# GewelsJI/MVLT

Measured on AMD Instinct MI355X. Metric: image-text pairs/sec/node, PVT-tiny MVLT pre-train step, higher is better.
Workload: dtype bf16

## Files before the change

### include/mvlt_hip.h

```cpp
#ifndef MVLT_HIP_H
#define MVLT_HIP_H
#include <stdint.h>
#ifdef __cplusplus
extern "C" {
#endif

#define MVLT_DT_BF16 0
#define MVLT_DT_FP32 1

#define MVLT_ABI_VERSION 7
const char* mvlt_last_error(void);
int mvlt_abi_version(void);
const char* mvlt_last_kernel(void);
int mvlt_sizeof(const char* name);

typedef struct mvlt_rowmap {
  int mode, rows_per_batch, batch_stride, offset;
  int r, w_in, tokens_in, hw_out, w_out, c_seg;
  int h_in;
} mvlt_rowmap;

typedef struct mvlt_gemm_nt_args {
  const void* A; const void* B; void* C;
  int M, N, K, lda, ldb, ldc;
  int dtype;
  int out_dtype;
  mvlt_rowmap a_map, c_map;
  const float* bias;
  int act;
  void* H;
  const float* row_scale;
  int rows_per_scale;
  const void* R;
  float* col_sum;
  float* col_sumsq;
  int col_copies;
  int split_k;
  void* post_y; int post_ld;
  const float* post_gamma; const float* post_beta; float post_eps;
  float* post_mean; float* post_rstd;
  int r_fp32;
} mvlt_gemm_nt_args;
int mvlt_gemm_nt(const mvlt_gemm_nt_args* args, void* stream);

typedef struct mvlt_gemm_tn_args {
  const void* A; const void* B; float* C;
  int M, N1, N2, lda, ldb, ldc;
  int dtype;
  mvlt_rowmap a_map, b_map;
  float* colsum_a;
  int splits;
  float* colsum_b;
  int trans_c;
  int c_taps, c_seg;
  const void* dgrad_wt; void* dgrad_out; int dgrad_ld;
  void* partials; long partials_bytes;
  int defer_fold;
  int c_overwrite;
} mvlt_gemm_tn_args;
int mvlt_gemm_tn(const mvlt_gemm_tn_args* args, void* stream);
int mvlt_tn_fold_flush(const void* partials, void* stream);
int mvlt_tn_fold_discard(const void* partials);

typedef struct mvlt_layernorm_args {
  const void* x; void* y;
  const float* gamma; const float* beta;
  float* mean; float* rstd;
  const float* add;
  int add_rows;
  int rows, C, ldx, ldy;
  mvlt_rowmap x_map, y_map;
  float eps;
  int dtype;
  int y_dtype;
  void* y2; const float* gamma2; const float* beta2; float eps2; float* mean2; float* rstd2;
} mvlt_layernorm_args;
int mvlt_layernorm_fwd(const mvlt_layernorm_args* args, void* stream);

typedef struct mvlt_layernorm_bwd_args {
  const void* dy; const void* x; void* dx;
  const float* gamma; const float* mean; const float* rstd;
  float* dgamma; float* dbeta;
  int rows, C, lddy, ldx, lddx;
  mvlt_rowmap dy_map, x_map, dx_map;
  int dx_accumulate;
  int dtype;
  int x_dtype, dx_dtype;
  void* dx2; const float* dx2_scale; int dx2_rows_per_scale; int lddx2;
  int dg_copies; long dg_copy_stride;
} mvlt_layernorm_bwd_args;
int mvlt_layernorm_bwd(const mvlt_layernorm_bwd_args* args, void* stream);
int mvlt_fold_copies(float* arena, int copies, long stride, const int* dst_index, int j0, int j1, float* dst, void* stream);

int mvlt_batch_sum(const void* in, float* out, int B, int R, int C, long batch_stride_rows, int ld, int dtype,
                   float* acc2 , int split, void* stream);

typedef struct mvlt_attn_args {
  const void* Q; const void* KV; void* O; float* lse;
  int B, H, N, M;
  int ldq, ldkv, ldo;
  int k_off, v_off;
  float scale;
  int dtype;
} mvlt_attn_args;
int mvlt_sr_attention_fwd(const mvlt_attn_args* args, void* stream);

typedef struct mvlt_attn_bwd_args {
  const void* Q; const void* KV; const void* O; const void* dO; const float* lse;
  void* dQ; void* dKV;
  int B, H, N, M;
  int ldq, ldkv, ldo, lddkv;
  int k_off, v_off;
  float scale;
  int dtype;
  int dkv_dtype;
} mvlt_attn_bwd_args;
int mvlt_sr_attention_bwd(const mvlt_attn_bwd_args* args, void* stream);
int mvlt_sr_attention_bwd_chunks(int B, int H, int N, int M, int dtype);
int mvlt_sr_attention_fwd_streamed(const mvlt_attn_args* args, void* stream);
int mvlt_sr_attention_bwd_streamed(const mvlt_attn_bwd_args* args, void* stream);


int mvlt_bert_embed_fwd(const long* ids, const float* word, const float* pos, const float* type0, const float* gamma,
                        const float* beta, const uint8_t* keep, float drop_p, void* y, float* mean, float* rstd,
                        int rows, int T, int hidden, float eps, int dtype, void* stream);
int mvlt_bert_embed_bwd(const void* dy, const long* ids, const float* word, const float* pos, const float* type0,
                        const float* gamma, const uint8_t* keep, float drop_p, const float* mean, const float* rstd,
                        float* dword, float* dpos, float* dtype0, float* dgamma, float* dbeta,
                        int rows, int T, int hidden, int dtype, void* stream);

int mvlt_patchify(const float* img, void* out, int B, int Cin, int H, int W, int k, int dtype, void* stream);

int mvlt_masked_select(const long* labels, int n, long ignore_index, int* idx, int* count, void* stream);

int mvlt_resize_bilinear_tokens(const float* in, int ld_in, float* out, int ld_out, int Hin, int Win, int Hout, int Wout, int C, int adjoint,
                                void* stream);
int mvlt_resize_bilinear_tokens_multi(const float* const* in, const int* ld_in, float* const* out, const int* ld_out, const int* Hin, const int* Win,
                                      const int* Hout, const int* Wout, const int* C, int count, int adjoint, void* stream);

int mvlt_gelu_bwd(const void* dy, const void* h, void* out, long n, int dtype, void* stream);
int mvlt_loss_compose(const float* const* losses, const float* weights, float* out, float* total, void* stream);

int mvlt_grid_mask_flags(uint8_t* flags, int B, int gh, int gw, int num_mask, int mode, uint64_t seed, uint64_t sample0, void* stream);
// ... 89 lines not shown
```

### mvlt_amd/_lib.py

```python
import ctypes as C
import os

import torch

_HERE = os.path.dirname(os.path.abspath(__file__))
LIB_PATH = os.environ.get("MVLT_HIP_LIB") or os.path.join(_HERE, "libmvlt_hip.so")


class MVLTError(RuntimeError):
    pass


if not os.path.exists(LIB_PATH):
    raise ImportError(f"{LIB_PATH} is missing: build it with `python -m mvlt_amd.build` (hipcc, gfx950). "
                      "mvlt_amd has no CPU or eager fallback.")
lib = C.CDLL(LIB_PATH)

c_int, c_float, c_void_p, c_long = C.c_int, C.c_float, C.c_void_p, C.c_long


class RowMap(C.Structure):
    _fields_ = [(n, c_int) for n in ("mode", "rows_per_batch", "batch_stride", "offset",
                                     "r", "w_in", "tokens_in", "hw_out", "w_out", "c_seg", "h_in")]


class GemmNTArgs(C.Structure):
    _fields_ = [("A", c_void_p), ("B", c_void_p), ("C", c_void_p),
                ("M", c_int), ("N", c_int), ("K", c_int), ("lda", c_int), ("ldb", c_int), ("ldc", c_int),
                ("dtype", c_int), ("out_dtype", c_int),
                ("a_map", RowMap), ("c_map", RowMap),
                ("bias", c_void_p), ("act", c_int), ("H", c_void_p),
                ("row_scale", c_void_p), ("rows_per_scale", c_int), ("R", c_void_p),
                ("col_sum", c_void_p), ("col_sumsq", c_void_p), ("col_copies", c_int), ("split_k", c_int),
                ("post_y", c_void_p), ("post_ld", c_int), ("post_gamma", c_void_p), ("post_beta", c_void_p), ("post_eps", C.c_float),
                ("post_mean", c_void_p), ("post_rstd", c_void_p), ("r_fp32", c_int)]


class PrepDesc(C.Structure):
    _fields_ = [("src", c_void_p), ("dst", c_void_p), ("kind", c_int), ("R", c_int), ("C", c_int), ("ld_out", c_int),
                ("d0", c_int), ("d1", c_int), ("d2", c_int), ("src_off", c_int), ("ss0", c_int), ("ss1", c_int), ("ss2", c_int),
                ("ds0", c_int), ("ds1", c_int), ("ds2", c_int)]


class GemmTNArgs(C.Structure):
    _fields_ = [("A", c_void_p), ("B", c_void_p), ("C", c_void_p),
                ("M", c_int), ("N1", c_int), ("N2", c_int), ("lda", c_int), ("ldb", c_int), ("ldc", c_int),
                ("dtype", c_int), ("a_map", RowMap), ("b_map", RowMap),
                ("colsum_a", c_void_p), ("splits", c_int), ("colsum_b", c_void_p), ("trans_c", c_int),
                ("c_taps", c_int), ("c_seg", c_int), ("dgrad_wt", c_void_p), ("dgrad_out", c_void_p), ("dgrad_ld", c_int),
                ("partials", c_void_p), ("partials_bytes", c_long), ("defer_fold", c_int), ("c_overwrite", c_int)]


class LayerNormArgs(C.Structure):
    _fields_ = [("x", c_void_p), ("y", c_void_p), ("gamma", c_void_p), ("beta", c_void_p),
                ("mean", c_void_p), ("rstd", c_void_p), ("add", c_void_p), ("add_rows", c_int),
                ("rows", c_int), ("C", c_int), ("ldx", c_int), ("ldy", c_int),
                ("x_map", RowMap), ("y_map", RowMap), ("eps", c_float), ("dtype", c_int), ("y_dtype", c_int),
                ("y2", c_void_p), ("gamma2", c_void_p), ("beta2", c_void_p), ("eps2", c_float), ("mean2", c_void_p), ("rstd2", c_void_p)]


class LayerNormBwdArgs(C.Structure):
    _fields_ = [("dy", c_void_p), ("x", c_void_p), ("dx", c_void_p),
                ("gamma", c_void_p), ("mean", c_void_p), ("rstd", c_void_p),
                ("dgamma", c_void_p), ("dbeta", c_void_p),
                ("rows", c_int), ("C", c_int), ("lddy", c_int), ("ldx", c_int), ("lddx", c_int),
                ("dy_map", RowMap), ("x_map", RowMap), ("dx_map", RowMap),
                ("dx_accumulate", c_int), ("dtype", c_int), ("x_dtype", c_int), ("dx_dtype", c_int),
                ("dx2", c_void_p), ("dx2_scale", c_void_p), ("dx2_rows_per_scale", c_int), ("lddx2", c_int),
                ("dg_copies", c_int), ("dg_copy_stride", C.c_long)]


class AttnArgs(C.Structure):
    _fields_ = [("Q", c_void_p), ("KV", c_void_p), ("O", c_void_p), ("lse", c_void_p),
                ("B", c_int), ("H", c_int), ("N", c_int), ("M", c_int),
                ("ldq", c_int), ("ldkv", c_int), ("ldo", c_int), ("k_off", c_int), ("v_off", c_int),
                ("scale", c_float), ("dtype", c_int)]


class AttnBwdArgs(C.Structure):
    _fields_ = [("Q", c_void_p), ("KV", c_void_p), ("O", c_void_p), ("dO", c_void_p), ("lse", c_void_p),
                ("dQ", c_void_p), ("dKV", c_void_p),
                ("B", c_int), ("H", c_int), ("N", c_int), ("M", c_int),
                ("ldq", c_int), ("ldkv", c_int), ("ldo", c_int), ("lddkv", c_int),
                ("k_off", c_int), ("v_off", c_int), ("scale", c_float), ("dtype", c_int), ("dkv_dtype", c_int)]


class MlpArgs(C.Structure):
    _fields_ = [("x", c_void_p), ("dy", c_void_p), ("w1", c_void_p), ("wb", c_void_p), ("wc", c_void_p),
                ("b1", c_void_p), ("b2", c_void_p), ("residual", c_void_p), ("row_scale", c_void_p), ("rows_per_scale", c_int),
                ("out", c_void_p), ("h_out", c_void_p), ("dw1", c_void_p), ("db1", c_void_p), ("dw2", c_void_p), ("db2", c_void_p),
                ("M", c_int), ("C", c_int), ("hid", c_int),
                ("ln_x", c_void_p), ("ln_gamma", c_void_p), ("ln_beta", c_void_p), ("ln_eps", c_float),
                ("ln_y", c_void_p), ("ln_mean", c_void_p), ("ln_rstd", c_void_p), ("out_op", c_void_p),
                ("post_gamma", c_void_p), ("post_beta", c_void_p), ("post_eps", c_float),
                ("post_y", c_void_p), ("post_mean", c_void_p), ("post_rstd", c_void_p),
                ("lnb_x", c_void_p), ("lnb_mean", c_void_p), ("lnb_rstd", c_void_p), ("lnb_gamma", c_void_p),
                ("lnb_dx", c_void_p), ("lnb_dx2", c_void_p), ("lnb_dx2_scale", c_void_p), ("lnb_dx2_rows_per_scale", c_int),
                ("lnb_partials", c_void_p), ("partials", c_void_p), ("partials_bytes", c_long), ("defer_fold", c_int)]


lib.mvlt_last_error.restype = C.c_char_p
lib.mvlt_last_kernel.restype = C.c_char_p
lib.mvlt_sizeof.argtypes = [C.c_char_p]
ABI_VERSION = 7
if lib.mvlt_abi_version() != ABI_VERSION:
    raise ImportError(f"ABI mismatch: {LIB_PATH} is version {lib.mvlt_abi_version()}, the binding is version {ABI_VERSION} (stale build? run python -m mvlt_amd.build)")
for _name, _cls in (("mvlt_rowmap", RowMap), ("mvlt_prep_desc", PrepDesc), ("mvlt_gemm_nt_args", GemmNTArgs), ("mvlt_gemm_tn_args", GemmTNArgs),
                    ("mvlt_layernorm_args", LayerNormArgs), ("mvlt_layernorm_bwd_args", LayerNormBwdArgs),
                    ("mvlt_attn_args", AttnArgs), ("mvlt_attn_bwd_args", AttnBwdArgs), ("mvlt_mlp_args", MlpArgs)):
    _n = lib.mvlt_sizeof(_name.encode())
    if _n != C.sizeof(_cls):
        raise ImportError(f"ABI mismatch for {_name}: library says {_n} bytes, binding has {C.sizeof(_cls)}")

EXPORTS = ["mvlt_last_error", "mvlt_last_kernel", "mvlt_abi_version", "mvlt_sizeof", "mvlt_gemm_nt", "mvlt_gemm_tn",
           "mvlt_layernorm_fwd", "mvlt_layernorm_bwd", "mvlt_fold_copies", "mvlt_batch_sum", "mvlt_sr_attention_fwd", "mvlt_sr_attention_bwd",
           "mvlt_bert_embed_fwd", "mvlt_bert_embed_bwd", "mvlt_patchify", "mvlt_masked_select", "mvlt_gather_rows",
           "mvlt_scatter_rows", "mvlt_cross_entropy_fwd", "mvlt_cross_entropy_bwd", "mvlt_adamw_step", "mvlt_smooth_l1_fwd", "mvlt_smooth_l1_bwd", "mvlt_cast_bf16",
           "mvlt_transpose_cast", "mvlt_row_scale", "mvlt_head_grad_prep", "mvlt_weight_prep", "mvlt_col_stats", "mvlt_bn_finalize", "mvlt_bn_finalize_norm", "mvlt_bn_norm", "mvlt_bn_bwd_reduce", "mvlt_bn_bwd_apply", "mvlt_ew_mul3_bwd",
           "mvlt_ew_mul", "mvlt_upsample_fwd", "mvlt_upsample_bwd", "mvlt_mlp_fwd", "mvlt_mlp_bwd_dx", "mvlt_mlp_bwd_dw",
           "mvlt_grid_mask_flags", "mvlt_grid_mask_apply", "mvlt_token_mask", "mvlt_resize_bilinear_tokens", "mvlt_resize_bilinear_tokens_multi", "mvlt_gelu_bwd",
           "mvlt_keep_mask", "mvlt_droppath_scales", "mvlt_loss_compose", "mvlt_add_column_sums",
           "mvlt_upsample_l1_fwd", "mvlt_upsample_l1_bwd", "mvlt_tn_fold_flush", "mvlt_tn_fold_discard", "mvlt_sr_attention_bwd_chunks",
           "mvlt_sr_attention_fwd_streamed", "mvlt_sr_attention_bwd_streamed"]

DT = {torch.bfloat16: 0, torch.float32: 1}


def last_kernel():
    s = lib.mvlt_last_kernel().decode()
    s = s.replace("(anonymous namespace)::", "")
    if s.startswith("void "):
        s = s[5:]
    depth = 0
    for i, ch in enumerate(s):
        depth += ch == "<"
        depth -= ch == ">"
        if ch == "(" and depth == 0:
            return s[:i]
    return s


def check(rc, what):
    if rc != 0:
        raise MVLTError(f"{what} failed ({rc}): {lib.mvlt_last_error().decode()}")


_raw_stream, _cur_device = torch._C._cuda_getCurrentRawStream, torch._C._cuda_getDevice


def stream_ptr():
    return c_void_p(_raw_stream(_cur_device()))


def ptr(t):
    if t is None:
        return None
    if not t.is_cuda:
        raise MVLTError("mvlt_amd ops need CUDA/HIP tensors (no CPU fallback)")
    return c_void_p(t.data_ptr())


def rowmap(rows_per_batch=0, batch_stride=0, offset=0):
    return RowMap(0, rows_per_batch, batch_stride, offset, 0, 0, 0, 0, 0, 0, 0)


def patchmap(r, w_in, tokens_in, hw_out, w_out, c_seg):
    return RowMap(1, 0, 0, 0, r, w_in, tokens_in, hw_out, w_out, c_seg, 0)


def conv3map(h, w, tokens_in, c_seg):
    return RowMap(2, 0, 0, 0, 3, w, tokens_in, h * w, w, c_seg, h)
```

### mvlt_amd/csrc/gemm.hip

```cpp
#ifndef MVLT_GELU_POLY
#define MVLT_GELU_POLY 3
#endif
#include "common.h"
#include <type_traits>
#include <map>
#include <mutex>
#ifndef MVLT_NT_EARLY_DEFAULT
#define MVLT_NT_EARLY_DEFAULT 0x100
#endif
#ifndef MVLT_ABL
#define MVLT_ABL 0
#endif
#ifndef MVLT_TN_EARLY
#define MVLT_TN_EARLY 0
#endif
#include "../../include/mvlt_hip.h"

namespace {

constexpr int BM = 128;
constexpr int NTHREADS = 256;
constexpr int ROW_BYTES = 128;
constexpr int CHUNKS = 8;

// ... 913 lines not shown
  if (do_colsum_b) {
    if (B_IT * NTHREADS == B_UNITS || tid < B_UNITS) {
      int c = tid % B_CH;
#pragma unroll
      for (int e = 0; e < PC; ++e) atomicAdd(&s_colsum[c * PC + e], colsum_local_b[e]);
    }
    __syncthreads();
    if (tid < BN && n2_0 + tid < p.N2) atomicAdd(&p.colsum_b[n2_0 + tid], s_colsum[tid]);
  }
#pragma unroll
  for (int i = 0; i < 4; ++i)
#pragma unroll
    for (int j = 0; j < TN_; ++j)
#pragma unroll
      for (int r = 0; r < 4; ++r) {
        int n1 = n1_0 + wm * 64 + i * 16 + 4 * fg + r;
        int n2 = n2_0 + wn * WN + j * 16 + fr;
        if (n1 < p.N1 && n2 < p.N2) atomicAdd(p.trans_c ? &p.C[(long)n2 * p.ldc + n1] : &p.C[(long)n1 * p.ldc + tn_dst_col(p, n2)], acc[i][j][r]);
      }
}

struct RowIt { int b, y, x; };
struct RowStep { int w, h, db, dy, dx; };
__device__ __forceinline__ RowStep row_step(const RowMap& rm, int delta) {
  RowStep s;
  if (rm.mode == 0) {
    if (rm.rows_per_batch == 0) { s.w = 0x7fffffff; s.h = 1; s.db = 0; s.dy = 0; s.dx = delta; }
    else { s.w = rm.rows_per_batch; s.h = 1; s.db = delta / s.w; s.dy = 0; s.dx = delta - s.db * s.w; }
  } else {
    s.w = rm.w_out; s.h = rm.hw_out / rm.w_out;
    s.db = delta / rm.hw_out;
    int rem = delta - s.db * rm.hw_out;
    s.dy = rem / s.w; s.dx = rem - s.dy * s.w;
  }
  return s;
}
__device__ __forceinline__ RowIt row_init(const RowMap& rm, int m) {
  RowIt it;
  if (rm.mode == 0) {
    if (rm.rows_per_batch == 0) { it.b = 0; it.y = 0; it.x = m; }
    else { it.b = m / rm.rows_per_batch; it.y = 0; it.x = m - it.b * rm.rows_per_batch; }
  } else {
    it.b = m / rm.hw_out;
    int rem = m - it.b * rm.hw_out;
    it.y = rem / rm.w_out; it.x = rem - it.y * rm.w_out;
  }
  return it;
}
__device__ __forceinline__ void row_advance(RowIt& it, const RowStep& s) {
  it.x += s.dx;
  int c = it.x >= s.w;
  it.x -= c ? s.w : 0;
  it.y += s.dy + c;
  int c2 = it.y >= s.h;
  it.y -= c2 ? s.h : 0;
  it.b += s.db + c2;
}
template <int MODE>
__device__ __forceinline__ bool row_phys(const RowMap& rm, const RowIt& it, int tap_dy, int tap_dx, int seg_rows, int& phys) {
  if constexpr (MODE == 0) {
    phys = it.b * rm.batch_stride + rm.offset + it.x;
    return true;
  } else if constexpr (MODE == 1) {
    phys = it.b * rm.tokens_in + (it.y * rm.r) * rm.w_in + it.x * rm.r + seg_rows;
    return true;
  } else {
    int y = it.y + tap_dy, x = it.x + tap_dx;
    phys = it.b * rm.tokens_in + y * rm.w_in + x;
    return (unsigned)y < (unsigned)rm.h_in && (unsigned)x < (unsigned)rm.w_in;
  }
}

template <int W> struct DmaTile {
  static constexpr int CH = W / 8, RPP = NTHREADS / CH, IT = TBK / RPP, ROWB = W * 2, BYTES = TBK * ROWB;
  static __device__ __forceinline__ int h(int row) {
    return W == 128 ? ((row & 3) | (((row >> 3) & 1) << 2)) : (((row >> 1) & 1) | (((row >> 3) & 1) << 1));
  }
  static __device__ __forceinline__ int frag_off(int frow, int window, int L) {
    return frow * ROWB + ((window ^ h(frow)) << 5) + ((L & 3) << 3);
  }
};

template <int BMT, int BN, int BMODE, int NS, bool DG = false>
__global__ __launch_bounds__(NTHREADS, 2) void gemm_tn_dma_kernel(mvlt_gemm_tn_args p, int m_per_split, int t1, int t2, int splits, bf16* part = nullptr) {
  using TA = DmaTile<BMT>;
  using TB = DmaTile<BN>;
  static_assert(!DG || (BMODE == 3 && BMT == BN && !MVLT_TN_EARLY), "dgrad rides on the plain-row single-tile kernels");
  constexpr int WM = BMT / 2, TM_ = WM / 16;
  constexpr int WN = BN / 2, TN_ = WN / 16;
  constexpr int STAGE = TA::BYTES + TB::BYTES;
  constexpr int LPT = TA::IT + TB::IT;
  extern __shared__ __attribute__((aligned(16))) char smem[];

  const int txy = t1 * t2;
  int bz, xy;
  if (splits >= 8) {
    const int xcd = blockIdx.x & 7, kq = blockIdx.x >> 3;
    const int zq = kq / txy;
    xy = kq - zq * txy;
    bz = zq * 8 + xcd;
    if (bz >= splits) return;
  } else {
    bz = blockIdx.x / txy;
    xy = blockIdx.x - bz * txy;
  }
  const int bx = xy % t1, by = xy / t1;

  const int tid = threadIdx.x, lane = tid & 63, wave = __builtin_amdgcn_readfirstlane(tid >> 6);
  const int wm = wave >> 1, wn = wave & 1;
  const int n1_0 = bx * BMT, n2_0 = by * BN;
  const unsigned smem_lds = (unsigned)(uintptr_t)smem;
  const int m_begin = bz * m_per_split;
  const int m_end = min(p.M, m_begin + m_per_split);
  const RowMap amap = to_rowmap(p.a_map), bmap = to_rowmap(p.b_map);
  const bool do_colsum = p.colsum_a != nullptr;
  const bool do_colsum_b = p.colsum_b != nullptr;

  const int a_row0 = tid / TA::CH;
  const int a_col = n1_0 + ((((tid % TA::CH)) ^ (TA::h(a_row0) << 1)) << 3);
  const bool a_col_ok = a_col < p.N1;
  const int b_row0 = tid / TB::CH;
  const int b_colg = n2_0 + ((((tid % TB::CH)) ^ (TB::h(b_row0) << 1)) << 3);
  const bool b_col_ok = b_colg < p.N2;
  int b_col = b_colg, b_seg_rows = 0, tap_dy = 0, tap_dx = 0;
  if constexpr (BMODE == 1 || BMODE == 2) {
    const int b_seg = b_colg / bmap.c_seg;
    b_col = b_colg - b_seg * bmap.c_seg;
    if constexpr (BMODE == 1) b_seg_rows = rowmap_seg(bmap, b_seg);
    else { tap_dy = b_seg / 3 - 1; tap_dx = b_seg - (b_seg / 3) * 3 - 1; }
  }
  const char* zsrc = (const char*)g_zero_page + ((tid * 16 + (blockIdx.x & 15) * 4096) & 65535);
  const char* a_src = (const char*)p.A + 2 * a_col;
  const char* b_src = (const char*)p.B + 2 * b_col;
  const unsigned a_rowb = 2u * (unsigned)p.lda, b_rowb = 2u * (unsigned)p.ldb;
  const RowStep astep = row_step(amap, TBK), bstep = row_step(bmap, TBK);
  RowIt ait[TA::IT], bit[TB::IT];
#pragma unroll
  for (int j = 0; j < TA::IT; ++j) ait[j] = row_init(amap, m_begin + j * TA::RPP + a_row0);
#pragma unroll
  for (int j = 0; j < TB::IT; ++j) bit[j] = row_init(bmap, m_begin + j * TB::RPP + b_row0);

  constexpr bool PLAIN = (BMODE == 3);
  const char* a_ptr[TA::IT];
  const char* b_ptr[TB::IT];
  const long a_adv = a_col_ok ? (long)TBK * a_rowb : 0, b_adv = b_col_ok ? (long)TBK * b_rowb : 0;
  if constexpr (PLAIN) {
#pragma unroll
    for (int j = 0; j < TA::IT; ++j) a_ptr[j] = a_col_ok ? a_src + (unsigned long long)(unsigned)(m_begin + j * TA::RPP + a_row0) * a_rowb : zsrc;
#pragma unroll
    for (int j = 0; j < TB::IT; ++j) b_ptr[j] = b_col_ok ? b_src + (unsigned long long)(unsigned)(m_begin + j * TB::RPP + b_row0) * b_rowb : zsrc;
  }
  auto issue = [&](int mt, int slot) {
    if constexpr (PLAIN) {
      const bool whole = mt + TBK <= m_end;
#pragma unroll
      for (int j = 0; j < TA::IT; ++j) {
        const int woff = slot * STAGE + (j * NTHREADS + wave * 64) * 16;
        const char* src = (whole || mt + j * TA::RPP + a_row0 < m_end) ? a_ptr[j] : zsrc;
        glds16(src, __builtin_amdgcn_readfirstlane(smem_lds + woff));
        a_ptr[j] += a_adv;
      }
#pragma unroll
      for (int j = 0; j < TB::IT; ++j) {
        const int woff = slot * STAGE + TA::BYTES + (j * NTHREADS + wave * 64) * 16;
        const char* src = (whole || mt + j * TB::RPP + b_row0 < m_end) ? b_ptr[j] : zsrc;
        glds16(src, __builtin_amdgcn_readfirstlane(smem_lds + woff));
        b_ptr[j] += b_adv;
      }
      return;
    }
#pragma unroll
    for (int j = 0; j < TA::IT; ++j) {
      int m = mt + j * TA::RPP + a_row0;
      int phys;
      bool ok = row_phys<0>(amap, ait[j], 0, 0, 0, phys) && m < m_end && a_col_ok;
      row_advance(ait[j], astep);
      const int woff = slot * STAGE + (j * NTHREADS + wave * 64) * 16;
      glds16(ok ? a_src + (unsigned long long)(unsigned)phys * a_rowb : zsrc, __builtin_amdgcn_readfirstlane(smem_lds + woff));
    }
#pragma unroll
    for (int j = 0; j < TB::IT; ++j) {
      int m = mt + j * TB::RPP + b_row0;
      int phys;
      bool ok = row_phys<(BMODE == 3 ? 0 : BMODE)>(bmap, bit[j], tap_dy, tap_dx, b_seg_rows, phys) && m < m_end && b_col_ok;
      row_advance(bit[j], bstep);
      const int woff = slot * STAGE + TA::BYTES + (j * NTHREADS + wave * 64) * 16;
      glds16(ok ? b_src + (unsigned long long)(unsigned)phys * b_rowb : zsrc, __builtin_amdgcn_readfirstlane(smem_lds + woff));
    }
  };

  const int g = lane >> 4, L = lane & 15;
  const int frow = 8 * g + (L >> 2);
  int aoff[TM_], boff[TN_];
#pragma unroll
  for (int i = 0; i < TM_; ++i) aoff[i] = TA::frag_off(frow, wm * TM_ + i, L);
#pragma unroll
  for (int j = 0; j < TN_; ++j) boff[j] = TB::frag_off(frow, wn * TN_ + j, L);

  f32x4 acc[TM_][TN_];
#pragma unroll
  for (int i = 0; i < TM_; ++i)
#pragma unroll
    for (int j = 0; j < TN_; ++j) acc[i][j] = f32x4{0.f, 0.f, 0.f, 0.f};
  f32x4 cs[2] = {f32x4{0.f, 0.f, 0.f, 0.f}, f32x4{0.f, 0.f, 0.f, 0.f}};
  const u32x4 ones = {0x3F803F80u, 0x3F803F80u, 0x3F803F80u, 0x3F803F80u};
  bf16* const nb = nullptr;
  constexpr int DGN = DG ? BN / 64 : 1, DGK = BMT / 32;
  u32x4 wtf[DGN][DGK];
  bf16* const sdX = (bf16*)(smem + NS * STAGE);
  if constexpr (DG) {
#pragma unroll
    for (int jn = 0; jn < DGN; ++jn)
#pragma unroll
      for (int ks = 0; ks < DGK; ++ks)
// ... 99 lines not shown
  if constexpr (DG) {
    asm volatile("s_waitcnt lgkmcnt(0)" ::: "memory");
    __syncthreads();
    if (m_end > m_begin) dg_store(m_begin + ((m_end - m_begin - 1) / TBK) * TBK);
    __syncthreads();
  }

  const int fr = lane & 15, fg = lane >> 4;
  if (do_colsum || do_colsum_b) {
    float* s_cs = (float*)smem;
    __syncthreads();
    if (do_colsum && fr == 0) {
#pragma unroll
      for (int t = 0; t < TM_ / 2; ++t)
#pragma unroll
        for (int r = 0; r < 4; ++r) s_cs[wm * WM + (wn * (TM_ / 2) + t) * 16 + 4 * fg + r] = cs[t][r];
    }
    if (do_colsum_b && fg == 0) {
#pragma unroll
      for (int t = 0; t < TN_ / 2; ++t) s_cs[wn * WN + (wm * (TN_ / 2) + t) * 16 + fr] = cs[t][0];
    }
    __syncthreads();
    if (do_colsum && tid < BMT && n1_0 + tid < p.N1) atomicAdd(&p.colsum_a[n1_0 + tid], s_cs[tid]);
    if (do_colsum_b && tid < BN && n2_0 + tid < p.N2) atomicAdd(&p.colsum_b[n2_0 + tid], s_cs[tid]);
  }
  if (part) {
    constexpr int LDP = WN + 8;
    __syncthreads();
    bf16* const st = (bf16*)smem + wave * 16 * LDP;
    bf16* const P = part + (size_t)bz * p.N1 * p.N2;
#pragma unroll
    for (int i = 0; i < TM_; ++i) {
      __builtin_amdgcn_wave_barrier();
#pragma unroll
      for (int j = 0; j < TN_; ++j)
#pragma unroll
        for (int r = 0; r < 4; ++r) st[(4 * fg + r) * LDP + j * 16 + fr] = (bf16)acc[i][j][r];
      __builtin_amdgcn_fence(__ATOMIC_RELEASE, "wavefront");
      __builtin_amdgcn_wave_barrier();
      __builtin_amdgcn_fence(__ATOMIC_ACQUIRE, "wavefront");
#pragma unroll
      for (int q = lane; q < 16 * (WN / 8); q += 64) {
        const int row = q / (WN / 8), ch = q - row * (WN / 8);
        const int n1 = n1_0 + wm * WM + i * 16 + row, n2 = n2_0 + wn * WN + ch * 8;
        if (n1 < p.N1 && n2 < p.N2) st_g<MVLT_NT_GEMM>((u32x4*)(P + (size_t)n1 * p.N2 + n2), *(const u32x4*)(st + row * LDP + ch * 8));
      }
    }
    return;
  }
  if (p.c_overwrite) {
    constexpr int LDP = WN + 4;
    constexpr int CPR = WN / 4;
    __syncthreads();
    float* const st = (float*)smem + wave * 16 * LDP;
#pragma unroll
    for (int i = 0; i < TM_; ++i) {
      __builtin_amdgcn_wave_barrier();
#pragma unroll
      for (int j = 0; j < TN_; ++j)
#pragma unroll
        for (int r = 0; r < 4; ++r) st[(4 * fg + r) * LDP + j * 16 + fr] = acc[i][j][r];
      __builtin_amdgcn_fence(__ATOMIC_RELEASE, "wavefront");
      __builtin_amdgcn_wave_barrier();
      __builtin_amdgcn_fence(__ATOMIC_ACQUIRE, "wavefront");
#pragma unroll
      for (int q = lane; q < 16 * CPR; q += 64) {
        const int row = q / CPR, ch = q - row * CPR;
        const int n1 = n1_0 + wm * WM + i * 16 + row, n2 = n2_0 + wn * WN + ch * 4;
        if (n1 < p.N1 && n2 < p.N2) st_g<MVLT_NT_GEMM>((f32x4*)(p.C + (size_t)n1 * p.ldc + n2), *(const f32x4*)(st + row * LDP + ch * 4));
      }
    }
    return;
  }
#pragma unroll
  for (int i = 0; i < TM_; ++i)
#pragma unroll
    for (int j = 0; j < TN_; ++j)
#pragma unroll
      for (int r = 0; r < 4; ++r) {
        int n1 = n1_0 + wm * WM + i * 16 + 4 * fg + r;
        int n2 = n2_0 + wn * WN + j * 16 + fr;
        if (n1 < p.N1 && n2 < p.N2) atomicAdd(p.trans_c ? &p.C[(long)n2 * p.ldc + n1] : &p.C[(long)n1 * p.ldc + tn_dst_col(p, n2)], acc[i][j][r]);
      }
}

template <int W>
__global__ __launch_bounds__(NTHREADS, 2) void conv3_wgrad_kernel(mvlt_gemm_tn_args p, int tiles_per_split, int n_o, int n_c, int splits, bf16* part) {
  using TA = DmaTile<64>;
  constexpr int R = 64 / W;
  constexpr int HW2 = W + 2, HR = (R + 2) * HW2;
  constexpr int H_IT = (HR * 8 + NTHREADS - 1) / NTHREADS;
  constexpr int HALO_BYTES = H_IT * NTHREADS * 16;
  constexpr int STAGE = TA::BYTES + HALO_BYTES;
  extern __shared__ __attribute__((aligned(16))) char smem[];
  const int txy = n_o * n_c;
  int bz, xy;
  if (splits >= 8) {
    const int xcd = blockIdx.x & 7, kq = blockIdx.x >> 3;
    const int zq = kq / txy;
    xy = kq - zq * txy;
    bz = zq * 8 + xcd;
    if (bz >= splits) return;
  } else {
    bz = blockIdx.x / txy;
    xy = blockIdx.x - bz * txy;
  }
  const int bo = xy % n_o, bc = xy / n_o;
  const int o0 = bo * 64, c0 = bc * 64;
  const int tid = threadIdx.x, lane = tid & 63, wave = __builtin_amdgcn_readfirstlane(tid >> 6);
  const int wm = wave >> 1, wn = wave & 1;
  const unsigned smem_lds = (unsigned)(uintptr_t)smem;
  const int ntiles = p.M / 64;
  const int t_begin = bz * tiles_per_split, t_end = min(ntiles, t_begin + tiles_per_split);
  const int Himg = p.b_map.h_in, cin = p.b_map.c_seg, tokens_in = p.b_map.tokens_in;
  const int tiles_per_img = Himg * W / 64;
  const char* zsrc = (const char*)g_zero_page + ((tid * 16 + (blockIdx.x & 15) * 4096) & 65535);

  const int a_row0 = tid / TA::CH;
  const int a_col = o0 + (((tid % TA::CH) ^ (TA::h(a_row0) << 1)) << 3);
  const char* a_src = (const char*)p.A + 2 * a_col;
  const unsigned a_rowb = 2u * (unsigned)p.lda, b_rowb = 2u * (unsigned)p.ldb;
  auto hh = [](int row) { return (row >> 1) & 1; };
  int h_dy[H_IT], h_off[H_IT];
  bool h_xok[H_IT];
#pragma unroll
  for (int j = 0; j < H_IT; ++j) {
    const int q = tid + j * NTHREADS, hr = q >> 3, sl = q & 7;
    const int hy = hr / HW2, hx = hr - hy * HW2;
    h_dy[j] = hy - 1;
    h_xok[j] = hr < HR && (unsigned)(hx - 1) < (unsigned)W;
    h_off[j] = (hx - 1) * (int)b_rowb + 2 * (c0 + ((sl ^ (hh(hr) << 1)) << 3));
  }
  auto issue = [&](int tile, int slot) {
    const int img = tile / tiles_per_img, y0 = (tile - img * tiles_per_img) * R;
#pragma unroll
    for (int j = 0; j < TA::IT; ++j) {
      const unsigned m = (unsigned)(tile * 64 + j * TA::RPP + a_row0);
      glds16(a_src + (unsigned long long)m * a_rowb, __builtin_amdgcn_readfirstlane(smem_lds + slot * STAGE + (j * NTHREADS + wave * 64) * 16));
    }
    const char* img_base = (const char*)p.B + (unsigned long long)(unsigned)(img * tokens_in) * b_rowb;
#pragma unroll
    for (int j = 0; j < H_IT; ++j) {
      const int y = y0 + h_dy[j];
      const bool ok = h_xok[j] && (unsigned)y < (unsigned)Himg;
      glds16(ok ? img_base + (long)(y * W) * (long)b_rowb + h_off[j] : zsrc,
             __builtin_amdgcn_readfirstlane(smem_lds + slot * STAGE + TA::BYTES + (j * NTHREADS + wave * 64) * 16));
    }
  };

  const int g = lane >> 4, L = lane & 15;
  const int frow = 8 * g + (L >> 2);
  int aoff[2];
#pragma unroll
  for (int i = 0; i < 2; ++i) aoff[i] = TA::frag_off(frow, wm * 2 + i, L);
  int boff[2][9];
#pragma unroll
  for (int ks = 0; ks < 2; ++ks) {
    const int pix = ks * 32 + frow, py = pix / W, px = pix - py * W;
#pragma unroll
    for (int t = 0; t < 9; ++t) {
      const int hr = (py + t / 3) * HW2 + px + t % 3;
      boff[ks][t] = TA::BYTES + hr * 128 + (((wn * 2) ^ hh(hr)) << 5) + ((L & 3) << 3);
    }
  }
  f32x4 acc[2][9][2];
#pragma unroll
// ... 73 lines not shown
__global__ void tn_fold_kernel(const bf16* __restrict__ part, int splits, int N1, int N2, float* __restrict__ C, int ldc);

constexpr int FOLD_MAX = 32;
struct FoldDesc { const bf16* part; float* C; int splits, N1, N2, ldc, wg0; };
struct FoldBatch { FoldDesc d[FOLD_MAX]; int n, total_wgs; };
__global__ void tn_fold_multi_kernel(FoldBatch b);
struct FoldPending {
  FoldBatch b = {};
  long used = 0;
  hipStream_t stream = nullptr;
  hipEvent_t ev = nullptr;
};
std::mutex g_fold_mu;
std::map<const void*, FoldPending> g_fold;
int fold_wgs(const FoldDesc& d) { return (int)(((long)d.N1 * d.N2 / 8 + 31) / 32); }
void fold_flush_locked(FoldPending& f, hipStream_t reader, bool order_reader) {
  if (f.b.n > 0) {
    f.b.total_wgs = f.b.d[f.b.n - 1].wg0 + fold_wgs(f.b.d[f.b.n - 1]);
    MVLT_LAUNCH(tn_fold_multi_kernel, dim3((unsigned)f.b.total_wgs), dim3(256), 0, f.stream, f.b);
    if (order_reader && reader != f.stream) {
      if (!f.ev) (void)hipEventCreateWithFlags(&f.ev, hipEventDisableTiming);
      if (f.ev && hipEventRecord(f.ev, f.stream) == hipSuccess) (void)hipStreamWaitEvent(reader, f.ev, 0);
    }
  }
  f.b.n = 0;
  f.used = 0;
}
bf16* fold_acquire(const mvlt_gemm_tn_args& a, long need, hipStream_t s, int room = 1) {
  if (!a.partials || ((uintptr_t)a.partials & 15) || need > a.partials_bytes) return nullptr;
  std::lock_guard<std::mutex> lk(g_fold_mu);
  FoldPending& f = g_fold[a.partials];
  bool flush = f.b.n > 0 && (!a.defer_fold || f.stream != s || f.b.n + room > FOLD_MAX || f.used + need > a.partials_bytes);
  const float* c_lo = a.C;
  const float* c_hi = a.C + (size_t)(a.N1 - 1) * a.ldc + a.N2;
  for (int i = 0; i < f.b.n && !flush; ++i) {
    const FoldDesc& d = f.b.d[i];
    const float* d_lo = d.C;
    const float* d_hi = d.C + (size_t)(d.N1 - 1) * d.ldc + d.N2;
    if (c_lo < d_hi && d_lo < c_hi) flush = true;
  }
  if (flush) fold_flush_locked(f, s, true);
  f.stream = s;
  if (!a.defer_fold) return (bf16*)a.partials;
  return (bf16*)((char*)a.partials + f.used);
}
void fold_launch(const mvlt_gemm_tn_args& a, const bf16* part, int splits, hipStream_t s) {
  const long groups = (long)a.N1 * a.N2 / 8;
  if (!a.defer_fold) {
    MVLT_LAUNCH(tn_fold_kernel, dim3((unsigned)((groups + 31) / 32)), dim3(256), 0, s, part, splits, a.N1, a.N2, a.C, a.ldc);
    return;
  }
  std::lock_guard<std::mutex> lk(g_fold_mu);
  FoldPending& f = g_fold[a.partials];
  FoldDesc& d = f.b.d[f.b.n];
  d.part = part; d.C = a.C; d.splits = splits; d.N1 = a.N1; d.N2 = a.N2; d.ldc = a.ldc;
  d.wg0 = f.b.n == 0 ? 0 : f.b.d[f.b.n - 1].wg0 + fold_wgs(f.b.d[f.b.n - 1]);
  ++f.b.n;
  f.used += ((long)splits * a.N1 * a.N2 * 2 + 255) & ~255L;
}

template <int W> int launch_conv3_wgrad(const mvlt_gemm_tn_args& a, hipStream_t s) {
  constexpr int R = 64 / W, HR = (R + 2) * (W + 2), H_IT = (HR * 8 + NTHREADS - 1) / NTHREADS;
  const size_t lds = (size_t)2 * (DmaTile<64>::BYTES + H_IT * NTHREADS * 16);
  const int n_o = a.N1 / 64, n_c = a.b_map.c_seg / 64, ntiles = a.M / 64;
  static const int min_tiles = getenv("MVLT_CONV_WGRAD_MINT") ? atoi(getenv("MVLT_CONV_WGRAD_MINT")) : 16;
  int splits = (512 + n_o * n_c - 1) / (n_o * n_c);
  if (splits > ntiles / min_tiles) splits = ntiles / min_tiles;
  if (splits < 1) splits = 1;
  if (splits >= 8) splits = (splits + 4) / 8 * 8;
  if (splits > ntiles) splits = ntiles;
  const int tps = (ntiles + splits - 1) / splits;
  splits = (ntiles + tps - 1) / tps;
  dim3 grid((unsigned)((splits >= 8 ? 8 * ((splits + 7) / 8) : splits) * n_o * n_c)), block(NTHREADS);
  mvlt_max_lds<(conv3_wgrad_kernel<W>)>();
  static const bool part_ok = !(getenv("MVLT_TN_P8") && atoi(getenv("MVLT_TN_P8")) == 0);
  bf16* const part = (part_ok && a.partials && splits >= 4 && a.ldc % 4 == 0 && ((uintptr_t)a.C & 15) == 0 && lds >= (size_t)4 * 16 * (9 * 32 + 8) * 2)
                         ? fold_acquire(a, (long)splits * a.N1 * a.N2 * 2, s) : nullptr;
  MVLT_LAUNCH((conv3_wgrad_kernel<W>), grid, block, lds, s, a, tps, n_o, n_c, splits, part);
  if (part) fold_launch(a, part, splits, s);
  return mvlt_check_launch("mvlt_gemm_tn");
}

template <int BN, int AMODE, int EPI, int BK, int BMT = BM>
__global__ __launch_bounds__(NTHREADS, BMT == 256 ? 2 : 1) void gemm_nt_dma_kernel(mvlt_gemm_nt_args p, int ns_flags) {
  const int ns = ns_flags & 0xff;
  const bool early = (ns_flags & 0x100) != 0;
  constexpr int ROWB = BK * 2;
  constexpr int CH = BK / 8;
  constexpr int RPL = NTHREADS / CH;
  constexpr int WN = BN / 2, TN_ = WN / 16;
  constexpr int WM = BMT / 2, TM_ = WM / 16;
  constexpr int A_ITERS = BMT * CH / NTHREADS;
  constexpr int B_ITERS = BN * CH / NTHREADS;
  constexpr int LPT = A_ITERS + B_ITERS;
  constexpr int STAGE = (BMT + BN) * ROWB;
  auto swzk = [](int row, int chunk) { return CH == 8 ? (chunk ^ ((row >> 1) & 7)) : (chunk ^ ((0 - (row >> 2)) & 3)); };
  extern __shared__ __attribute__((aligned(16))) char smem[];

  const int tid = threadIdx.x, lane = tid & 63, wave = __builtin_amdgcn_readfirstlane(tid >> 6);
  const int wm = wave >> 1, wn = wave & 1;
  const int tiles_m = (p.M + BMT - 1) / BMT;
  const int tiles_n = (p.N + BN - 1) / BN;
  const int bid = blockIdx.x;
  const int xcd = bid & 7, bslot = bid >> 3;
  const int tile_m = (bslot / tiles_n) * 8 + xcd, tile_n = bslot % tiles_n;
  if (tile_m >= tiles_m) return;
  const int m0 = tile_m * BMT, n0 = tile_n * BN;
  const RowMap amap = to_rowmap(p.a_map);
  const unsigned smem_lds = (unsigned)(uintptr_t)smem;
#ifdef MVLT_NT_STAGGER
  if constexpr (EPI == 3 || EPI == 4) {
    if (bid < 1024) {
      const int phase = (bid >> MVLT_NT_STAGGER) & 3;
      for (int q = 0; q < phase; ++q) __builtin_amdgcn_s_sleep(127);
    }
  }
#endif

  const int row_in = tid / CH;
  const int chunk = swzk(row_in, tid % CH);
  const char* zsrc = (const char*)g_zero_page + ((tid * 16 + (bid & 15) * 4096) & 65535);

  const char* a_ptr[A_ITERS];
  bool a_ok[A_ITERS];
  int a_y[A_ITERS], a_x[A_ITERS];
#pragma unroll
  for (int i = 0; i < A_ITERS; ++i) {
    int m = m0 + row_in + RPL * i;
    a_ok[i] = m < p.M;
    RowIt it = row_init(amap, a_ok[i] ? m : 0);
    int phys;
    if constexpr (AMODE == 0) phys = it.b * amap.batch_stride + amap.offset + it.x;
    else if constexpr (AMODE == 1) phys = it.b * amap.tokens_in + (it.y * amap.r) * amap.w_in + it.x * amap.r;
    else phys = it.b * amap.tokens_in + it.y * amap.w_in + it.x;
    a_y[i] = it.y; a_x[i] = it.x;
    a_ptr[i] = (const char*)p.A + (unsigned long long)(unsigned)phys * (2u * (unsigned)p.lda);
  }
  const char* b_ptr[B_ITERS];
  bool b_ok[B_ITERS];
#pragma unroll
  for (int i = 0; i < B_ITERS; ++i) {
    int n = n0 + row_in + RPL * i;
    b_ok[i] = n < p.N;
    b_ptr[i] = (const char*)p.B + (unsigned long long)(unsigned)(b_ok[i] ? n : 0) * (2u * (unsigned)p.ldb);
  }

  const int nk_all = (p.K + BK - 1) / BK;
  const int nsplit = p.split_k > 1 ? p.split_k : 1;
  const int kt_per = (nk_all + nsplit - 1) / nsplit;
  const int kt0 = blockIdx.y * kt_per;
  int kpos = kt0 * BK + chunk * 8, seg = 0, kk = kpos;
  if constexpr (AMODE != 0) { seg = kk / amap.c_seg; kk -= seg * amap.c_seg; }
  auto issue = [&](int slot) {
    const bool k_ok = kpos < p.K;
    int off_bytes = (AMODE == 0 ? kpos : kk) * 2, tdy = 0, tdx = 0;
    if constexpr (AMODE == 1) off_bytes += rowmap_seg(amap, seg) * (2 * p.lda);
    if constexpr (AMODE == 2) {
      const int dy = seg / 3;
      tdy = dy - 1; tdx = seg - dy * 3 - 1;
      off_bytes += (tdy * amap.w_in + tdx) * (2 * p.lda);
    }
    if (MVLT_ABL == 1) { kpos += BK; return; }
#pragma unroll
    for (int i = 0; i < A_ITERS; ++i) {
      bool ok = a_ok[i] && k_ok;
      if constexpr (AMODE == 2) ok = ok && (unsigned)(a_y[i] + tdy) < (unsigned)amap.h_in && (unsigned)(a_x[i] + tdx) < (unsigned)amap.w_in;
      if (MVLT_ABL == 4) ok = false;
      glds16(ok ? a_ptr[i] + off_bytes : zsrc, __builtin_amdgcn_readfirstlane(smem_lds + slot * STAGE + (i * NTHREADS + wave * 64) * 16));
    }
#pragma unroll
    for (int i = 0; i < B_ITERS; ++i)
      glds16((b_ok[i] && k_ok && MVLT_ABL != 4) ? b_ptr[i] + kpos * 2 : zsrc,
             __builtin_amdgcn_readfirstlane(smem_lds + slot * STAGE + BMT * ROWB + (i * NTHREADS + wave * 64) * 16));
    kpos += BK;
    if constexpr (AMODE != 0) {
      kk += BK;
      while (kk >= amap.c_seg) { kk -= amap.c_seg; ++seg; }
    }
  };

  f32x4 acc[TM_][TN_];
#pragma unroll
  for (int i = 0; i < TM_; ++i)
#pragma unroll
    for (int j = 0; j < TN_; ++j) acc[i][j] = f32x4{0.f, 0.f, 0.f, 0.f};

  const int nk = min(kt_per, nk_all - kt0);
  if (nk <= 0) return;
  const int fr = lane & 15, fg = lane >> 4;
  for (int st = 0; st < (early ? ns : ns - 1) && st < nk; ++st) issue(st);
  if (ns == 1 && !early) issue(0);
  int slot = 0, islot = early ? 0 : ns - 1;
  for (int kt = 0; kt < nk; ++kt) {
    const int ahead = min(nk - 1 - kt, early ? ns - 1 : ns - 2);
    if (ahead >= 4) asm volatile("s_waitcnt vmcnt(%0) lgkmcnt(0)" ::"n"(4 * LPT) : "memory");
    else if (ahead == 3) asm volatile("s_waitcnt vmcnt(%0) lgkmcnt(0)" ::"n"(3 * LPT) : "memory");
    else if (ahead == 2) asm volatile("s_waitcnt vmcnt(%0) lgkmcnt(0)" ::"n"(2 * LPT) : "memory");
    else if (ahead == 1) asm volatile("s_waitcnt vmcnt(%0) lgkmcnt(0)" ::"n"(LPT) : "memory");
    else asm volatile("s_waitcnt vmcnt(0) lgkmcnt(0)" ::: "memory");
    __builtin_amdgcn_s_barrier();
    asm volatile("" ::: "memory");
    if (!early) {
      if (ns > 1 && kt + ns - 1 < nk) issue(islot);
      islot = islot + 1 >= ns ? 0 : islot + 1;
    }
    const char* a_s = smem + slot * STAGE + (wm * WM) * ROWB;
    const char* b_s = smem + slot * STAGE + BMT * ROWB + (wn * WN) * ROWB;
    slot = slot + 1 >= ns ? 0 : slot + 1;
    constexpr int KS = BK / 32;
    u32x4 fa[KS][TM_], fb[KS][TN_];
#pragma unroll
    for (int ks = 0; ks < KS; ++ks) {
#pragma unroll
      for (int i = 0; i < TM_; ++i) {
        int r = i * 16 + fr;
        fa[ks][i] = MVLT_ABL == 3 ? u32x4{(unsigned)r, 1u, 2u, 3u} : *(const u32x4*)(a_s + r * ROWB + swzk(wm * WM + r, ks * 4 + fg) * 16);
      }
#pragma unroll
      for (int j = 0; j < TN_; ++j) {
        int r = j * 16 + fr;
        fb[ks][j] = MVLT_ABL == 3 ? u32x4{(unsigned)r, 5u, 6u, 7u} : *(const u32x4*)(b_s + r * ROWB + swzk(wn * WN + r, ks * 4 + fg) * 16);
      }
    }
    if (early) {
      asm volatile("s_waitcnt lgkmcnt(0)" ::: "memory");
      __builtin_amdgcn_s_barrier();
      asm volatile("" ::: "memory");
      if (kt + ns < nk) issue(islot);
      islot = islot + 1 >= ns ? 0 : islot + 1;
    }
#pragma unroll
    for (int ks = 0; ks < KS; ++ks) {
      __builtin_amdgcn_sched_barrier(0);
      if (MVLT_ABL == 2) {
#pragma unroll
        for (int i = 0; i < TM_; ++i) acc[i][0][0] += __builtin_bit_cast(float, fa[ks][i][0] ^ fb[ks][i % TN_][1]);
        continue;
      }
#pragma unroll
      for (int i = 0; i < TM_; ++i)
#pragma unroll
        for (int j = 0; j < TN_; ++j) mma16(acc[i][j], fa[ks][i], fa[ks][i], fb[ks][j], fb[ks][j], (bf16*)nullptr);
    }
  }
  __syncthreads();
  static_assert(BMT == BM || (BN != 192 && EPI != 0), "the 256-row tile carries the lean epilogues only");
  if constexpr (BN == 192) nt_epilogue_192<EPI>(p, acc, smem, m0, n0, wave, lane);
  else if constexpr (EPI == 0) nt_epilogue<bf16, BN>(p, acc, smem, m0, n0, wave, lane);
  else nt_epilogue_lean<BN, EPI, TM_>(p, acc, smem, m0, n0, wave, lane);
}

__device__ __forceinline__ void glds16_s(const char* sbase, unsigned voff, unsigned dst) {
  unsigned keep;
  asm volatile("s_mov_b32 %0, m0\n\ts_mov_b32 m0, %3\n\ts_nop 0\n\tglobal_load_lds_dwordx4 %1, %2\n\ts_mov_b32 m0, %0"
               : "=&s"(keep) : "v"(voff), "s"(sbase), "s"(dst) : "memory");
}
#define MVLT_BAR()                                  \
  do {                                              \
    __builtin_amdgcn_sched_barrier(0);              \
    __builtin_amdgcn_s_barrier();                   \
    asm volatile("" ::: "memory");                  \
    __builtin_amdgcn_sched_barrier(0);              \
  } while (0)
template <int N> __device__ __forceinline__ void wait_vm() { asm volatile("s_waitcnt vmcnt(%0)" ::"n"(N) : "memory"); }
template <int N> __device__ __forceinline__ void wait_lgkm() { asm volatile("s_waitcnt lgkmcnt(%0)" ::"n"(N) : "memory"); }

template <int EPI, int TM, bool CHK = false>
__device__ __forceinline__ void nt_epilogue_w80(const mvlt_gemm_nt_args& p, f32x4 (&acc)[TM][5], char* smem, int m0, int n0, int wave, int lane) {
  static_assert(EPI == 1 || EPI == 2, "the 80-column wave tile carries the plain and the residual epilogue");
  constexpr int WN = 80, LDW = WN + 4, NH = TM / 2, NIT = 5;
  const int wm = wave >> 2, wn = wave & 3;
  const int fr = lane & 15, fg = lane >> 4;
  const int ofp32 = p.out_dtype;
  const int rfp32 = ofp32 | p.r_fp32;
  float* stage = (float*)smem + wave * 32 * LDW;
  const int rpb = p.c_map.rows_per_batch;
  const float inv_rpb = rpb > 0 ? 1.0f / (float)rpb : 0.f;
  const float inv_rps = (EPI == 2 && p.rows_per_scale > 0) ? 1.0f / (float)p.rows_per_scale : 0.f;
  int rl[NIT], cc[NIT];
#pragma unroll
  for (int it = 0; it < NIT; ++it) {
    const int sidx = it * 64 + lane;
    rl[it] = sidx / 10;
    cc[it] = (sidx - rl[it] * 10) * 8;
  }
  long idx[2][NIT];
  float rs[2][NIT];
  u32x4 raw[2][NIT][2];
  auto request = [&](int half) {
    const int sl = half & 1;
#pragma unroll
    for (int it = 0; it < NIT; ++it) {
      const int m = CHK ? min(m0 + wm * (TM * 16) + half * 32 + rl[it], p.M - 1) : m0 + wm * (TM * 16) + half * 32 + rl[it];
      long phys = m;
      if (rpb > 0) {
        const int b = fdiv24(m, rpb, inv_rpb);
        phys = (long)b * p.c_map.batch_stride + p.c_map.offset + (m - b * rpb);
      }
      idx[sl][it] = phys * p.ldc + n0 + wn * WN + cc[it];
      rs[sl][it] = 1.0f;
      if (EPI == 2) {
        if (p.row_scale) rs[sl][it] = p.row_scale[fdiv24(m, p.rows_per_scale, inv_rps)];
        if (rfp32) { raw[sl][it][0] = ld_g<MVLT_NT_LD>((const u32x4*)((const float*)p.R + idx[sl][it])); raw[sl][it][1] = ld_g<MVLT_NT_LD>((const u32x4*)((const float*)p.R + idx[sl][it] + 4)); }
        else raw[sl][it][0] = ld_g<MVLT_NT_LD>((const u32x4*)((const bf16*)p.R + idx[sl][it]));
      }
    }
  };
  request(0);
#pragma unroll
  for (int half = 0; half < NH; ++half) {
    const int sl = half & 1;
    __builtin_amdgcn_wave_barrier();
#pragma unroll
    for (int ii = 0; ii < 2; ++ii)
#pragma unroll
      for (int j = 0; j < 5; ++j)
#pragma unroll
        for (int r = 0; r < 4; ++r) stage[(ii * 16 + 4 * fg + r) * LDW + j * 16 + fr] = acc[half * 2 + ii][j][r];
    if (half + 1 < NH) request(half + 1);
    __builtin_amdgcn_fence(__ATOMIC_RELEASE, "wavefront");
    __builtin_amdgcn_wave_barrier();
    __builtin_amdgcn_fence(__ATOMIC_ACQUIRE, "wavefront");
#pragma unroll
    for (int it = 0; it < NIT; ++it) {
      if (CHK && m0 + wm * (TM * 16) + half * 32 + rl[it] >= p.M) continue;
      const f32x4 v0 = *(const f32x4*)(stage + rl[it] * LDW + cc[it]), v1 = *(const f32x4*)(stage + rl[it] * LDW + cc[it] + 4);
      float v[8] = {v0[0], v0[1], v0[2], v0[3], v1[0], v1[1], v1[2], v1[3]};
      if (p.bias) {
        const f32x4 b0 = *(const f32x4*)(p.bias + n0 + wn * WN + cc[it]), b1 = *(const f32x4*)(p.bias + n0 + wn * WN + cc[it] + 4);
#pragma unroll
        for (int e = 0; e < 4; ++e) { v[e] += b0[e]; v[4 + e] += b1[e]; }
      }
// ... 674 lines not shown
      asm volatile("" ::: "memory");
      if (t + 1 < 9) issue_b(kc, t + 1, bslot ^ 1);
      else if (kc + 1 < nkc) issue_b(kc + 1, 0, bslot ^ 1);
      const int tapoff = (t / 3 - 1) * HW2 + (t % 3 - 1);
      const char* b_s = smem + HALO_BYTES + bslot * BSTAGE + (wn * WN) * ROWB;
      bslot ^= 1;
      u32x4 fa[2][TM_], fb[2][TN_];
#pragma unroll
      for (int i = 0; i < TM_; ++i) {
        const int hr = hbase[i] + tapoff;
        const char* rowp = smem + hr * 128;
        const int sw = swzh(hr);
#pragma unroll
        for (int ks = 0; ks < 2; ++ks) fa[ks][i] = *(const u32x4*)(rowp + (((ks * 4 + fg) ^ sw) << 4));
      }
#pragma unroll
      for (int ks = 0; ks < 2; ++ks)
#pragma unroll
        for (int j = 0; j < TN_; ++j) {
          int r = j * 16 + fr;
          fb[ks][j] = *(const u32x4*)(b_s + r * ROWB + swzk(wn * WN + r, ks * 4 + fg) * 16);
        }
#pragma unroll
      for (int ks = 0; ks < 2; ++ks) {
        __builtin_amdgcn_sched_barrier(0);
#pragma unroll
        for (int i = 0; i < TM_; ++i)
#pragma unroll
          for (int j = 0; j < TN_; ++j) mma16(acc[i][j], fa[ks][i], fa[ks][i], fb[ks][j], fb[ks][j], (bf16*)nullptr);
      }
    }
  }
  __syncthreads();
  if constexpr (BN == 192) nt_epilogue_192<EPI>(p, acc, smem, m0, n0, wave, lane);
  else nt_epilogue_lean<BN, EPI, TM_>(p, acc, smem, m0, n0, wave, lane);
}

template <int W, int BN, int EPI> void launch_conv3_nt(const mvlt_gemm_nt_args& a, hipStream_t s) {
  constexpr int R = BM / W, HR = (R + 2) * (W + 2), H_IT = (HR * 8 + NTHREADS - 1) / NTHREADS;
  size_t lds = (size_t)H_IT * NTHREADS * 16 + (size_t)2 * BN * ROW_BYTES;
  const size_t stage = (size_t)4 * 32 * (BN / 2 + 4) * sizeof(float);
  if (lds < stage) lds = stage;
  const int tiles_m = a.M / BM, tiles_n = (a.N + BN - 1) / BN;
  dim3 grid((unsigned)(8 * ((tiles_m + 7) / 8) * tiles_n)), block(NTHREADS);
  mvlt_max_lds<(conv3_nt_kernel<W, BN, EPI>)>();
  MVLT_LAUNCH((conv3_nt_kernel<W, BN, EPI>), grid, block, lds, s, a);
}
template <int W> bool dispatch_conv3_nt(const mvlt_gemm_nt_args& a, int epi, hipStream_t s) {
  const bool wide = a.N % 192 == 0 && a.N % 128 != 0 && (epi == 1 || epi == 5) && a.c_map.mode == 0;
  if (wide) { if (epi == 1) launch_conv3_nt<W, 192, 1>(a, s); else launch_conv3_nt<W, 192, 5>(a, s); return true; }
  if (a.N <= 64) {
    switch (epi) {
      case 1: launch_conv3_nt<W, 64, 1>(a, s); return true;
      case 2: launch_conv3_nt<W, 64, 2>(a, s); return true;
      case 5: launch_conv3_nt<W, 64, 5>(a, s); return true;
      default: return false;
    }
  }
  switch (epi) {
    case 1: launch_conv3_nt<W, 128, 1>(a, s); return true;
    case 2: launch_conv3_nt<W, 128, 2>(a, s); return true;
    case 5: launch_conv3_nt<W, 128, 5>(a, s); return true;
    default: return false;
  }
}

int check_rowmap(const mvlt_rowmap& m, const char* who) {
  if (m.mode == 0) {
    MVLT_REQUIRE(m.rows_per_batch >= 0, "%s: rows_per_batch < 0", who);
  } else if (m.mode == 1) {
    MVLT_REQUIRE(m.r > 0 && m.w_in > 0 && m.tokens_in > 0 && m.hw_out > 0 && m.w_out > 0 && m.c_seg > 0 && m.c_seg % 16 == 0,
                 "%s: bad patch map (c_seg must be a positive multiple of 16)", who);
  } else if (m.mode == 2) {
    MVLT_REQUIRE(m.r == 3 && m.w_in > 0 && m.h_in > 0 && m.tokens_in >= m.h_in * m.w_in && m.hw_out == m.h_in * m.w_in &&
                 m.w_out == m.w_in && m.c_seg > 0 && m.c_seg % 8 == 0, "%s: bad 3x3 neighbourhood map", who);
  } else {
    MVLT_REQUIRE(false, "%s: unknown rowmap mode %d", who, m.mode);
  }
  return MVLT_OK;
}

}

extern "C" int mvlt_gemm_nt(const mvlt_gemm_nt_args* a, void* stream) {
  MVLT_REQUIRE(a && a->A && a->B && a->C, "mvlt_gemm_nt: null operand");
  MVLT_REQUIRE(a->M >= 0 && a->N > 0 && a->K > 0, "mvlt_gemm_nt: bad shape M=%d N=%d K=%d", a->M, a->N, a->K);
  MVLT_REQUIRE(a->dtype == 0 || a->dtype == 1, "mvlt_gemm_nt: dtype must be 0 (bf16) or 1 (fp32)");
  const int pc = a->dtype == 0 ? 8 : 4;
  MVLT_REQUIRE(a->K % pc == 0 && a->lda % pc == 0 && a->ldb % pc == 0, "mvlt_gemm_nt: K/lda/ldb must be multiples of %d elements (16 B)", pc);
  MVLT_REQUIRE(((uintptr_t)a->A & 15) == 0 && ((uintptr_t)a->B & 15) == 0, "mvlt_gemm_nt: A/B must be 16-byte aligned");
  MVLT_REQUIRE(a->act >= 0 && a->act <= 2, "mvlt_gemm_nt: bad act");
  MVLT_REQUIRE(a->act != 2 || a->H, "mvlt_gemm_nt: act=2 (gelu') needs H");
  MVLT_REQUIRE(!a->row_scale || a->rows_per_scale > 0, "mvlt_gemm_nt: row_scale needs rows_per_scale");
  MVLT_REQUIRE((a->col_sum == nullptr) == (a->col_sumsq == nullptr), "mvlt_gemm_nt: col_sum and col_sumsq come together");
  MVLT_REQUIRE(a->split_k <= 1 || (a->dtype == 0 && a->out_dtype == 1 && a->act == 0 && !a->H && !a->R && !a->row_scale && !a->col_sum &&
                                   a->c_map.mode == 0 && a->split_k <= 64),
               "mvlt_gemm_nt: split_k needs bf16 operands, fp32 C (zeroed by the caller) and a plain epilogue (A may be gathered)");
  MVLT_REQUIRE(a->col_copies >= 0, "mvlt_gemm_nt: col_copies < 0");
  MVLT_REQUIRE(!a->r_fp32 || (a->R && a->R != a->C && a->dtype == 0 && a->out_dtype == 0 && a->act == 0 && !a->col_sum && !a->post_y && a->split_k <= 1 && a->c_map.mode == 0 &&
                              a->N % 8 == 0 && a->ldc % 8 == 0 && (((uintptr_t)a->C | (uintptr_t)a->R) & 15) == 0 && a->M < (1 << 24) && !getenv("MVLT_NT_GENERIC_EPI")),
               "mvlt_gemm_nt: r_fp32 (fp32 residual beside a bf16 C) exists in the residual epilogue of the bf16 LDS-DMA kernels only (plain c_map, N % 8 == 0, 16-byte aligned C / R)");
  MVLT_REQUIRE(a->out_dtype >= 0 && a->out_dtype <= 2, "mvlt_gemm_nt: out_dtype is 0 (bf16), 1 (fp32) or 2 (fp16, with col_sum only)");
  MVLT_REQUIRE(a->out_dtype != 2 || (a->dtype == 0 && a->col_sum && a->act == 0 && !a->R && !a->row_scale && a->split_k <= 1 && a->c_map.mode == 0 && a->N % 8 == 0 &&
                                     a->ldc % 8 == 0 && ((uintptr_t)a->C & 15) == 0 && a->M < (1 << 24) && !getenv("MVLT_NT_GENERIC_EPI")),
               "mvlt_gemm_nt: fp16 output exists in the column-statistics epilogue of the bf16 LDS-DMA kernels only (plain c_map, N % 8 == 0, 16-byte aligned C)");
  if (int e = check_rowmap(a->a_map, "mvlt_gemm_nt a_map")) return e;
  if (int e = check_rowmap(a->c_map, "mvlt_gemm_nt c_map")) return e;
  MVLT_REQUIRE(a->a_map.mode == 0 || a->K == a->a_map.r * a->a_map.r * a->a_map.c_seg, "mvlt_gemm_nt: gather K != r*r*c_seg");
  MVLT_REQUIRE(a->c_map.mode == 0 || a->N == a->c_map.r * a->c_map.r * a->c_map.c_seg, "mvlt_gemm_nt: scatter N != r*r*c_seg");
  MVLT_REQUIRE(a->c_map.mode != 2, "mvlt_gemm_nt: the 3x3 map is a gather only (its dgrad is a gather with flipped taps)");
  MVLT_REQUIRE(!a->post_y || (a->dtype == 0 && a->split_k <= 1),
               "mvlt_gemm_nt: post_y needs the bf16 LDS-DMA path (no fp32 operands, no split_k)");
  if (a->M == 0) return MVLT_OK;
  hipStream_t s = (hipStream_t)stream;
  const int tiles_m = (a->M + BM - 1) / BM;
  const bool narrow = a->N <= 64;
  const int bn = narrow ? 64 : 128;
  const int tiles_n = (a->N + bn - 1) / bn;
  const int bk = a->dtype == 0 ? 64 : 32;
  const int nbuf = a->K <= bk ? 1 : 2;
  size_t lds = (size_t)nbuf * (BM + bn) * ROW_BYTES;
  const size_t stage = (size_t)4 * 32 * (bn / 2 + 4) * sizeof(float);
  if (lds < stage) lds = stage;
  dim3 grid((unsigned)(8 * ((tiles_m + 7) / 8) * tiles_n), (unsigned)(a->split_k > 1 ? a->split_k : 1)), block(NTHREADS);
  if (a->dtype == 0) {
    const int nk = ((a->K + 63) / 64 + (a->split_k > 1 ? a->split_k : 1) - 1) / (a->split_k > 1 ? a->split_k : 1);
    int epi = 0;
    const bool plain_epi = a->act == 0 && !a->R && !a->row_scale && !a->col_sum && !a->H && a->c_map.mode == 0;
    const bool lean_ok = (a->c_map.mode == 0 || (a->c_map.mode == 1 && a->c_map.c_seg % 8 == 0)) && a->split_k <= 1 && (a->N % 8 == 0 || plain_epi) && a->ldc % 8 == 0 && ((uintptr_t)a->C & 15) == 0 &&
                         (!a->R || ((uintptr_t)a->R & 15) == 0) && (!a->H || ((uintptr_t)a->H & 15) == 0) && a->M < (1 << 24) &&
                         !getenv("MVLT_NT_GENERIC_EPI");
    if (lean_ok && a->c_map.mode == 1) {
      if (a->act == 0 && !a->col_sum && !a->R && !a->row_scale) epi = 6;
      else if (a->act == 0 && !a->col_sum && a->R) epi = 7;
    } else if (lean_ok) {
      if (a->act == 1 && !a->R && !a->row_scale && !a->col_sum && a->out_dtype == 0) epi = 3;
      else if (a->act == 2 && !a->R && !a->row_scale && !a->col_sum && a->out_dtype == 0) epi = 4;
      else if (a->act == 0 && a->R && !a->col_sum) epi = 2;
      else if (a->act == 0 && !a->R && !a->row_scale && a->col_sum) epi = 5;
      else if (a->act == 0 && !a->R && !a->row_scale && !a->col_sum) epi = 1;
    }
    const int bkd = (!narrow && a->a_map.mode == 0 && (epi == 3 || (epi == 4 && !getenv("MVLT_NT_EPI4_BK64"))) && a->K <= 512 && !getenv("MVLT_NT_BK64")) ? 32 : 64;
    const int nkd = bkd == 32 ? (a->K + 31) / 32 : nk;
    int ns = nkd < 2 ? nkd : 2;
    if (const char* e = getenv("MVLT_NT_NS")) { ns = atoi(e); if (ns > nkd) ns = nkd; if (ns < 2) ns = nkd < 2 ? nkd : 2; if (ns > 6) ns = 6; }
    size_t lds2 = (size_t)ns * (BM + bn) * (bkd * 2);
    if (lds2 < stage) lds2 = stage;
    static const int early_flag = getenv("MVLT_NT_EARLY") ? (atoi(getenv("MVLT_NT_EARLY")) ? 0x100 : 0) : MVLT_NT_EARLY_DEFAULT;
    const int ns_lds = ns;
    if (nkd >= 2) ns |= early_flag;
    if (a->post_y) {
      MVLT_REQUIRE(epi == 2 && a->N == bn && a->a_map.mode == 0 && a->c_map.mode == 0 && a->c_map.rows_per_batch == 0 && a->post_gamma && a->post_beta &&
                   a->post_mean && a->post_rstd && a->post_ld % 8 == 0 && ((uintptr_t)a->post_y & 15) == 0 && ((uintptr_t)a->post_gamma & 15) == 0,
                   "mvlt_gemm_nt: post_y needs bf16 operands, a residual (R), N == 64 or 128, identity row maps, 16-byte aligned outputs");
      if (lds2 < stage + 2048) lds2 = stage + 2048;
      if (narrow) MVLT_LAUNCH((gemm_nt_dma_kernel<64, 0, 8, 64>), grid, block, lds2, s, *a, ns);
      else MVLT_LAUNCH((gemm_nt_dma_kernel<128, 0, 8, 64>), grid, block, lds2, s, *a, ns);
      return mvlt_check_launch("mvlt_gemm_nt");
    }
#define MVLT_NT_LAUNCH_E(BN_, AM_, BK_)                                                                                 \
  do {                                                                                                               \
    switch (epi) {                                                                                                   \
      case 1: MVLT_LAUNCH((gemm_nt_dma_kernel<BN_, AM_, 1, BK_>), grid, block, lds2, s, *a, ns); break;            \
      case 2: MVLT_LAUNCH((gemm_nt_dma_kernel<BN_, AM_, 2, BK_>), grid, block, lds2, s, *a, ns); break;            \
      case 3: MVLT_LAUNCH((gemm_nt_dma_kernel<BN_, AM_, 3, BK_>), grid, block, lds2, s, *a, ns); break;            \
      case 4: MVLT_LAUNCH((gemm_nt_dma_kernel<BN_, AM_, 4, BK_>), grid, block, lds2, s, *a, ns); break;            \
      case 5: MVLT_LAUNCH((gemm_nt_dma_kernel<BN_, AM_, 5, BK_>), grid, block, lds2, s, *a, ns); break;            \
      case 6: MVLT_LAUNCH((gemm_nt_dma_kernel<BN_, AM_, 6, BK_>), grid, block, lds2, s, *a, ns); break;            \
      case 7: MVLT_LAUNCH((gemm_nt_dma_kernel<BN_, AM_, 7, BK_>), grid, block, lds2, s, *a, ns); break;            \
      default: MVLT_LAUNCH((gemm_nt_dma_kernel<BN_, AM_, 0, BK_>), grid, block, lds2, s, *a, ns);                  \
    }                                                                                                                \
  } while (0)
#define MVLT_NT_LAUNCH(BN_, BK_)                                                                                     \
  do {                                                                                                               \
    if (a->a_map.mode == 0) MVLT_NT_LAUNCH_E(BN_, 0, BK_);                                                           \
    else if (a->a_map.mode == 1) MVLT_NT_LAUNCH_E(BN_, 1, BK_);                                                      \
    else MVLT_NT_LAUNCH_E(BN_, 2, BK_);                                                                              \
  } while (0)
    static const bool conv_nt_ok = !getenv("MVLT_NO_CONV_NT");
    if (conv_nt_ok && a->a_map.mode == 2 && (epi == 1 || epi == 2 || epi == 5) && a->split_k <= 1 && a->a_map.c_seg % 64 == 0 && a->c_map.mode == 0 &&
        (a->a_map.w_in == 16 || a->a_map.w_in == 32 || a->a_map.w_in == 64) && (a->a_map.h_in * a->a_map.w_in) % BM == 0 && a->M % BM == 0 &&
        a->M % (a->a_map.h_in * a->a_map.w_in) == 0 && a->a_map.hw_out == a->a_map.h_in * a->a_map.w_in && a->a_map.w_out == a->a_map.w_in &&
        a->K == 9 * a->a_map.c_seg && a->lda >= a->a_map.c_seg && a->ldb >= a->K) {
      bool done = a->a_map.w_in == 32 ? dispatch_conv3_nt<32>(*a, epi, s) : a->a_map.w_in == 16 ? dispatch_conv3_nt<16>(*a, epi, s) : dispatch_conv3_nt<64>(*a, epi, s);
      if (done) return mvlt_check_launch("mvlt_gemm_nt");
    }
    static const int ntp8 = getenv("MVLT_NT_P8") ? atoi(getenv("MVLT_NT_P8")) : 15;
    if (ntp8 && a->a_map.mode == 0 && a->a_map.rows_per_batch == 0 && a->c_map.mode == 0 && epi >= 1 && epi <= 5 && a->K % 64 == 0 && a->K >= 128) {
      auto cost = [&](int bm, int bn) -> long {
        if (a->M % bm || a->N % bn) return 0;
        const long tiles = (long)(a->M / bm) * (a->N / bn);
        if (tiles < 192) return 0;
        return ((tiles + 255) / 256) * (long)bm * bn;
      };
      const long c256 = (ntp8 & 1) ? cost(256, 256) : 0, c192 = (ntp8 & 2) ? cost(192, 256) : 0;
      const long c320 = ((ntp8 & 4) && a->N % 256 != 0 && (epi == 1 || (epi == 2 && (a->K >= 640 || (ntp8 & 16))))) ? cost(192, 320) : 0;
      bool done = false;
      if (!c320 && !c256 && !c192 && epi == 1 && (ntp8 & 8) && (a->M % 256 || a->N % 256)) {
        const long tiles = (long)((a->M + 255) / 256) * ((a->N + 255) / 256);
        const long rounds = (tiles + 255) / 256;
        if (tiles >= 384 && (double)a->M * a->N >= 0.85 * (double)rounds * 256.0 * 65536.0) { launch_nt_p8<1, 4, 2, 2, true>(*a, s); done = true; }
      }
      if (!done && !c320 && !c256 && !c192 && (ntp8 & 4) && a->N % 320 == 0 && a->N % 256 != 0 && a->M % 192 != 0 && (epi == 1 || (epi == 2 && (a->K >= 640 || (ntp8 & 16))))) {
        const long tiles = (long)((a->M + 191) / 192) * (a->N / 320);
        const long rounds = (tiles + 255) / 256;
        if (tiles >= 192 && (double)a->M * a->N >= 0.85 * (double)rounds * 256.0 * 192.0 * 320.0) {
          if (epi == 1) launch_nt_p8<1, 3, 3, 2, true>(*a, s);
          else launch_nt_p8<2, 3, 3, 2, true>(*a, s);
          done = true;
        }
      }
      if (done) return mvlt_check_launch("mvlt_gemm_nt");
      if (c320) done = dispatch_nt_p8<3, 3, 2>(*a, epi, s);
      else if (c256 && (!c192 || c256 <= c192)) done = dispatch_nt_p8<4, 2, 2>(*a, epi, s);
      else if (c192) done = dispatch_nt_p8<3, 2, 2>(*a, epi, s);
      if (done) return mvlt_check_launch("mvlt_gemm_nt");
    }
    const bool wide = !narrow && a->N % 192 == 0 && a->N % 128 != 0 && (epi == 1 || epi == 5) && a->c_map.mode == 0 && a->a_map.mode != 1 &&
                      a->K >= 128 && !getenv("MVLT_NT_NO192");
    if (wide) {
      const int tn192 = a->N / 192;
      dim3 grid192((unsigned)(8 * ((tiles_m + 7) / 8) * tn192), 1);
      size_t lds3 = (size_t)ns_lds * (BM + 192) * ROW_BYTES;
      const size_t stage192 = (size_t)4 * 32 * 100 * sizeof(float);
      if (lds3 < stage192) lds3 = stage192;
      if (a->a_map.mode == 0 && epi == 1) MVLT_LAUNCH((gemm_nt_dma_kernel<192, 0, 1, 64>), grid192, block, lds3, s, *a, ns);
      else if (a->a_map.mode == 0) MVLT_LAUNCH((gemm_nt_dma_kernel<192, 0, 5, 64>), grid192, block, lds3, s, *a, ns);
      else if (epi == 1) MVLT_LAUNCH((gemm_nt_dma_kernel<192, 2, 1, 64>), grid192, block, lds3, s, *a, ns);
      else MVLT_LAUNCH((gemm_nt_dma_kernel<192, 2, 5, 64>), grid192, block, lds3, s, *a, ns);
    } else if (narrow) MVLT_NT_LAUNCH(64, 64);
    else if (bkd == 32 && epi == 3) MVLT_LAUNCH((gemm_nt_dma_kernel<128, 0, 3, 32>), grid, block, lds2, s, *a, ns);
    else if (bkd == 32) MVLT_LAUNCH((gemm_nt_dma_kernel<128, 0, 4, 32>), grid, block, lds2, s, *a, ns);
    else MVLT_NT_LAUNCH(128, 64);
#undef MVLT_NT_LAUNCH_E
#undef MVLT_NT_LAUNCH
  } else {
    if (narrow) MVLT_LAUNCH((gemm_nt_kernel<float, 64>), grid, block, lds, s, *a, nbuf);
    else MVLT_LAUNCH((gemm_nt_kernel<float, 128>), grid, block, lds, s, *a, nbuf);
  }
  return mvlt_check_launch("mvlt_gemm_nt");
}

bf16* mvlt_fold_acquire_ext(const mvlt_gemm_tn_args& a, long need, hipStream_t s, int descriptors) { return fold_acquire(a, need, s, descriptors); }
void mvlt_fold_launch_ext(const mvlt_gemm_tn_args& a, const bf16* part, int splits, hipStream_t s) { fold_launch(a, part, splits, s); }

extern "C" int mvlt_tn_fold_discard(const void* partials) {
  std::lock_guard<std::mutex> lk(g_fold_mu);
  for (auto& kv : g_fold)
    if (!partials || kv.first == partials) { kv.second.b.n = 0; kv.second.used = 0; }
  return MVLT_OK;
}

extern "C" int mvlt_tn_fold_flush(const void* partials, void* stream) {
  std::lock_guard<std::mutex> lk(g_fold_mu);
  for (auto& kv : g_fold)
    if (!partials || kv.first == partials) fold_flush_locked(kv.second, (hipStream_t)stream, true);
  return mvlt_check_launch("mvlt_tn_fold_flush");
}

extern "C" int mvlt_gemm_tn(const mvlt_gemm_tn_args* a, void* stream) {
  MVLT_REQUIRE(a && a->A && a->B && a->C, "mvlt_gemm_tn: null operand");
  MVLT_REQUIRE(a->M >= 0 && a->N1 > 0 && a->N2 > 0, "mvlt_gemm_tn: bad shape");
  MVLT_REQUIRE(a->dtype == 0 || a->dtype == 1, "mvlt_gemm_tn: dtype must be 0 (bf16) or 1 (fp32)");
  const int pc = a->dtype == 0 ? 8 : 4;
  MVLT_REQUIRE(a->lda % pc == 0 && a->ldb % pc == 0, "mvlt_gemm_tn: lda/ldb must be multiples of %d elements (16 B)", pc);
  MVLT_REQUIRE(a->lda >= (a->N1 + pc - 1) / pc * pc, "mvlt_gemm_tn: lda must cover N1 rounded up to %d", pc);
  MVLT_REQUIRE(a->b_map.mode != 0 || a->ldb >= (a->N2 + pc - 1) / pc * pc, "mvlt_gemm_tn: ldb must cover N2 rounded up to %d", pc);
  MVLT_REQUIRE(((uintptr_t)a->A & 15) == 0 && ((uintptr_t)a->B & 15) == 0, "mvlt_gemm_tn: A/B must be 16-byte aligned");
  if (int e = check_rowmap(a->a_map, "mvlt_gemm_tn a_map")) return e;
  if (int e = check_rowmap(a->b_map, "mvlt_gemm_tn b_map")) return e;
  MVLT_REQUIRE(a->a_map.mode == 0, "mvlt_gemm_tn: A cannot be a patch gather");
  MVLT_REQUIRE(!(a->colsum_a && a->colsum_b), "mvlt_gemm_tn: at most one of colsum_a / colsum_b");
  MVLT_REQUIRE(a->b_map.mode == 0 || a->N2 == a->b_map.r * a->b_map.r * a->b_map.c_seg, "mvlt_gemm_tn: gather N2 != r*r*c_seg");
  MVLT_REQUIRE(a->c_taps <= 1 || (a->trans_c == 0 && a->c_seg > 0 && a->N2 == a->c_taps * a->c_seg), "mvlt_gemm_tn: c_taps needs trans_c == 0 and N2 == c_taps*c_seg");
  MVLT_REQUIRE(!a->dgrad_out || (a->dtype == 0 && a->M < (1 << 24) && a->b_map.mode == 0 && a->a_map.mode == 0),
               "mvlt_gemm_tn: dgrad_out rides on the bf16 LDS-DMA kernel only (bf16 operands, M < 2^24, plain row maps): every other path would leave it unwritten");
  if (a->M == 0) return MVLT_OK;
  hipStream_t s = (hipStream_t)stream;
  const int mtiles = (a->M + TBK - 1) / TBK;
  static const bool conv_wgrad_ok = !getenv("MVLT_NO_CONV_WGRAD");
  if (conv_wgrad_ok && a->dtype == 0 && a->b_map.mode == 2 && a->a_map.mode == 0 && a->a_map.rows_per_batch == 0 && !a->trans_c && a->c_taps <= 1 &&
      !a->colsum_a && !a->colsum_b && a->N1 % 64 == 0 && a->b_map.c_seg % 64 == 0 && a->N2 == 9 * a->b_map.c_seg && a->M % 64 == 0 &&
      (a->b_map.w_in == 8 || a->b_map.w_in == 16 || a->b_map.w_in == 32 || a->b_map.w_in == 64) && (a->b_map.h_in * a->b_map.w_in) % 64 == 0 &&
      a->M % (a->b_map.h_in * a->b_map.w_in) == 0 && a->ldb >= a->b_map.c_seg) {
    hipStream_t s2 = (hipStream_t)stream;
    if (a->b_map.w_in == 64) return launch_conv3_wgrad<64>(*a, s2);
    if (a->b_map.w_in == 32) return launch_conv3_wgrad<32>(*a, s2);
    if (a->b_map.w_in == 16) return launch_conv3_wgrad<16>(*a, s2);
    return launch_conv3_wgrad<8>(*a, s2);
  }
  static const bool tnp8 = !(getenv("MVLT_TN_P8") && atoi(getenv("MVLT_TN_P8")) == 0);
  if (tnp8 && a->partials && a->dtype == 0 && a->a_map.mode == 0 && a->b_map.mode == 0 && a->a_map.rows_per_batch == 0 && a->b_map.rows_per_batch == 0 && a->c_taps <= 1 &&
      !a->trans_c && !a->dgrad_out && a->M % 64 == 0 && a->N1 % 256 == 0 && a->N2 % 256 == 0 && a->ldc % 4 == 0 && ((uintptr_t)a->C & 15) == 0 && ((uintptr_t)a->partials & 15) == 0) {
    const int tiles = (a->N1 / 256) * (a->N2 / 256), nkt = a->M / 64;
    if (tiles >= 16 && tiles <= 64 && nkt / (256 / tiles) >= 16 && a->partials_bytes >= (long)(256 / tiles) * a->N1 * a->N2 * 2)
      return launch_tn_p8_partial<4, 2, 2>(*a, s);
  }
  static const bool tn320 = !(getenv("MVLT_TN_P8_320") && atoi(getenv("MVLT_TN_P8_320")) == 0);
  if (tnp8 && tn320 && a->partials && a->dtype == 0 && a->a_map.mode == 0 && a->b_map.mode == 0 && a->a_map.rows_per_batch == 0 && a->b_map.rows_per_batch == 0 && a->c_taps <= 1 &&
      !a->trans_c && !a->dgrad_out && a->M % 64 == 0 && a->N1 % 8 == 0 && a->N2 % 8 == 0 && a->ldc % 4 == 0 && ((uintptr_t)a->C & 15) == 0 && ((uintptr_t)a->partials & 15) == 0 &&
      a->lda % 8 == 0 && a->ldb % 8 == 0 && (((uintptr_t)a->A | (uintptr_t)a->B) & 15) == 0) {
    const bool direct = a->N2 % 320 == 0 && a->N1 >= 1024, swapped = !direct && a->N1 % 320 == 0 && a->N2 >= 1024;
    if (direct || swapped) {
      const int rows = direct ? a->N1 : a->N2, cols = direct ? a->N2 : a->N1;
      const int tiles = ((rows + 191) / 192) * (cols / 320), nkt = a->M / 64;
      if (tiles >= 6 && tiles <= 16 && nkt / (256 / tiles) >= 16 && (double)rows >= 0.85 * 192.0 * ((rows + 191) / 192)) {
        const int rc = direct ? launch_tn_p8_320<false>(*a, s) : launch_tn_p8_320<true>(*a, s);
        if (rc <= 0) return rc;
      }
    }
  }
  if (a->dtype == 0 && a->M < (1 << 24)) {
    if (a->dgrad_out) {
      MVLT_REQUIRE(a->dgrad_wt && a->N1 == a->N2 && (a->N1 == 64 || a->N1 == 128) && a->a_map.rows_per_batch == 0 && a->b_map.mode == 0 &&
                   a->b_map.rows_per_batch == 0 && !a->trans_c && a->c_taps <= 1 && !a->colsum_b && a->dgrad_ld % 8 == 0 &&
                   (((uintptr_t)a->dgrad_out | (uintptr_t)a->dgrad_wt) & 15) == 0,
                   "mvlt_gemm_tn: dgrad_out needs bf16 operands, plain rows, N1 == N2 == 64 or 128, no transposed / tap output, 16-byte aligned buffers");
      int splits = a->splits > 0 ? a->splits : (a->N1 == 64 ? 256 : 384);
      static const int min_tiles = getenv("MVLT_TN_MINT") ? atoi(getenv("MVLT_TN_MINT")) : 8;
      if (min_tiles > 1 && splits > mtiles / min_tiles) splits = mtiles / min_tiles;
      if (splits >= 8) splits = (splits + 4) / 8 * 8;
      if (splits > mtiles) splits = mtiles;
      if (splits < 1) splits = 1;
      const int m_per_split = ((mtiles + splits - 1) / splits) * TBK;
      splits = (a->M + m_per_split - 1) / m_per_split;
      dim3 grid((unsigned)(splits >= 8 ? 8 * ((splits + 7) / 8) : splits)), block(NTHREADS);
      if (a->N1 == 64) {
        const size_t lds = (size_t)4 * TBK * 128 * 2 + 64 * 64 * 2;
        static bool once = (hipFuncSetAttribute((const void*)gemm_tn_dma_kernel<64, 64, 3, 4, true>, hipFuncAttributeMaxDynamicSharedMemorySize, (int)lds) == hipSuccess);
        (void)once;
        MVLT_LAUNCH((gemm_tn_dma_kernel<64, 64, 3, 4, true>), grid, block, lds, s, *a, m_per_split, 1, 1, splits, (bf16*)nullptr);
      } else {
        const size_t lds = (size_t)2 * TBK * 256 * 2 + 64 * 128 * 2;
        static bool once = (hipFuncSetAttribute((const void*)gemm_tn_dma_kernel<128, 128, 3, 2, true>, hipFuncAttributeMaxDynamicSharedMemorySize, (int)lds) == hipSuccess);
        (void)once;
        MVLT_LAUNCH((gemm_tn_dma_kernel<128, 128, 3, 2, true>), grid, block, lds, s, *a, m_per_split, 1, 1, splits, (bf16*)nullptr);
      }
      return mvlt_check_launch("mvlt_gemm_tn");
    }
    MVLT_REQUIRE(!a->c_overwrite || (!a->trans_c && a->c_taps <= 1 && a->N2 % 4 == 0 && a->ldc % 4 == 0 && ((uintptr_t)a->C & 15) == 0),
                 "mvlt_gemm_tn: c_overwrite needs the plain output layout, N2 % 4 == 0, ldc % 4 == 0 and a 16-byte aligned C");
    const bool small_out = a->N1 <= 128 && a->N2 <= 128 && !getenv("MVLT_TN_NO64");
    const int bmt = (a->N1 <= 64 || small_out) ? 64 : 128, bn = (a->N2 <= 64 || small_out) ? 64 : 128;
    const int t1 = (a->N1 + bmt - 1) / bmt, t2 = (a->N2 + bn - 1) / bn;
    int splits = a->c_overwrite ? 1 : a->splits;
    if (splits <= 0) {
      splits = ((t1 * t2 == 1 ? 384 : 512) + t1 * t2 - 1) / (t1 * t2);
      if (splits >= 8) splits = (splits + 4) / 8 * 8;
      if (splits > 4096) splits = 4096;
      static const int min_tiles = getenv("MVLT_TN_MINT") ? atoi(getenv("MVLT_TN_MINT")) : 8;
      if (min_tiles > 1 && splits > mtiles / min_tiles) splits = mtiles / min_tiles;
    }
    if (splits > mtiles) splits = mtiles;
    if (splits < 1) splits = 1;
    int m_per_split = ((mtiles + splits - 1) / splits) * TBK;
    splits = (a->M + m_per_split - 1) / m_per_split;
    const int ns = (bmt + bn == 256) ? 2 : (bmt + bn == 192) ? 3 : 4;
    const size_t lds = (size_t)ns * TBK * (bmt + bn) * 2;
    dim3 grid((unsigned)((splits >= 8 ? 8 * ((splits + 7) / 8) : splits) * t1 * t2)), block(NTHREADS);
    static const int part_min = getenv("MVLT_TN_PART_MIN") ? atoi(getenv("MVLT_TN_PART_MIN")) : 8;
    static const long part_min_out = getenv("MVLT_TN_PART_MINOUT") ? atol(getenv("MVLT_TN_PART_MINOUT")) : 16384;
    bf16* const part = (tnp8 && a->partials && !a->c_overwrite && splits >= part_min && !a->trans_c && a->c_taps <= 1 && a->N2 % 8 == 0 && a->ldc % 4 == 0 && ((uintptr_t)a->C & 15) == 0 &&
                        (long)a->N1 * a->N2 >= part_min_out)
                           ? fold_acquire(*a, (long)splits * a->N1 * a->N2 * 2, s) : nullptr;
#define MVLT_TN_LAUNCH(BMT_, BN_, NS_)                                                                                          \
  do {                                                                                                                         \
    if (a->b_map.mode == 0 && a->b_map.rows_per_batch == 0 && a->a_map.rows_per_batch == 0)                                                        \
      MVLT_LAUNCH((gemm_tn_dma_kernel<BMT_, BN_, 3, NS_>), grid, block, lds, s, *a, m_per_split, t1, t2, splits, part);                     \
    else if (a->b_map.mode == 0) MVLT_LAUNCH((gemm_tn_dma_kernel<BMT_, BN_, 0, NS_>), grid, block, lds, s, *a, m_per_split, t1, t2, splits, part); \
    else if (a->b_map.mode == 1) MVLT_LAUNCH((gemm_tn_dma_kernel<BMT_, BN_, 1, NS_>), grid, block, lds, s, *a, m_per_split, t1, t2, splits, part); \
    else MVLT_LAUNCH((gemm_tn_dma_kernel<BMT_, BN_, 2, NS_>), grid, block, lds, s, *a, m_per_split, t1, t2, splits, part);                   \
  } while (0)
    if (bmt == 128 && bn == 128) MVLT_TN_LAUNCH(128, 128, 2);
    else if (bmt == 128) MVLT_TN_LAUNCH(128, 64, 3);
    else if (bn == 128) MVLT_TN_LAUNCH(64, 128, 3);
    else MVLT_TN_LAUNCH(64, 64, 4);
#undef MVLT_TN_LAUNCH
    if (part) fold_launch(*a, part, splits, s);
    return mvlt_check_launch("mvlt_gemm_tn");
  }
  const bool narrow = a->N2 <= 64;
  const int bn = narrow ? 64 : 128;
  const int t1 = (a->N1 + BM - 1) / BM, t2 = (a->N2 + bn - 1) / bn;
  int splits = a->splits;
  if (splits <= 0) {
    splits = (1024 + t1 * t2 - 1) / (t1 * t2);
    if (splits > mtiles) splits = mtiles;
    if (splits > 4096) splits = 4096;
    if (splits < 1) splits = 1;
  }
  int m_per_split = ((mtiles + splits - 1) / splits) * TBK;
  splits = (a->M + m_per_split - 1) / m_per_split;
  const int rowb = a->dtype == 0 ? TElem<bf16>::ROWB : TElem<float>::ROWB;
  const size_t lds = (size_t)(BM + bn) * rowb + BM * sizeof(float);
  dim3 grid((unsigned)t1, (unsigned)t2, (unsigned)splits), block(NTHREADS);
  if (a->dtype == 0) {
    if (narrow) MVLT_LAUNCH((gemm_tn_kernel<bf16, 64>), grid, block, lds, s, *a, m_per_split);
    else MVLT_LAUNCH((gemm_tn_kernel<bf16, 128>), grid, block, lds, s, *a, m_per_split);
  } else {
    if (narrow) MVLT_LAUNCH((gemm_tn_kernel<float, 64>), grid, block, lds, s, *a, m_per_split);
    else MVLT_LAUNCH((gemm_tn_kernel<float, 128>), grid, block, lds, s, *a, m_per_split);
  }
  return mvlt_check_launch("mvlt_gemm_tn");
}
```

### mvlt_amd/csrc/runtime.hip

```cpp
#include "common.h"
#include "../../include/mvlt_hip.h"
#include <stdarg.h>
#include <stdlib.h>
#include <cxxabi.h>

static thread_local char g_err[512] = "";

void mvlt_set_error(const char* fmt, ...) {
  va_list ap;
  va_start(ap, fmt);
  vsnprintf(g_err, sizeof(g_err), fmt, ap);
  va_end(ap);
}

static thread_local hipError_t g_lds_err = hipSuccess;
void mvlt_note_lds_error(hipError_t e) { g_lds_err = e; }

int mvlt_check_launch(const char* what) {
  hipError_t e = hipGetLastError();
  if (e != hipSuccess) {
    if (g_lds_err != hipSuccess)
      mvlt_set_error("%s: launch failed: %s (raising the kernel's dynamic-LDS limit to 160 KB had failed on this device: %s)", what, hipGetErrorString(e), hipGetErrorString(g_lds_err));
    else
      mvlt_set_error("%s: launch failed: %s", what, hipGetErrorString(e));
    g_lds_err = hipSuccess;
    return MVLT_ERR_LAUNCH;
  }
  return MVLT_OK;
}

extern "C" const char* mvlt_last_error(void) { return g_err; }

static thread_local const void* g_last_kernel = nullptr;
static thread_local char g_last_kernel_name[512] = "";
void mvlt_note_kernel(const void* host_function) { g_last_kernel = host_function; }
extern "C" const char* mvlt_last_kernel(void) {
  g_last_kernel_name[0] = 0;
  if (!g_last_kernel) return g_last_kernel_name;
  const char* mangled = hipKernelNameRefByPtr(g_last_kernel, nullptr);
  if (!mangled) return g_last_kernel_name;
  int status = 0;
  char* dem = abi::__cxa_demangle(mangled, nullptr, nullptr, &status);
  snprintf(g_last_kernel_name, sizeof(g_last_kernel_name), "%s", (status == 0 && dem) ? dem : mangled);
  free(dem);
  return g_last_kernel_name;
}

extern "C" int mvlt_abi_version(void) { return MVLT_ABI_VERSION; }

extern "C" int mvlt_sizeof(const char* name) {
#define S(T) if (strcmp(name, #T) == 0) return (int)sizeof(T);
  S(mvlt_rowmap) S(mvlt_prep_desc) S(mvlt_gemm_nt_args) S(mvlt_gemm_tn_args) S(mvlt_layernorm_args) S(mvlt_layernorm_bwd_args)
  S(mvlt_attn_args) S(mvlt_attn_bwd_args) S(mvlt_mlp_args)
#undef S
  return -1;
}
```

### mvlt_amd/ops.py

```python
import ctypes as C

import torch

from . import _lib as L
from ._lib import DT, check, patchmap, ptr, rowmap, stream_ptr

_ID = rowmap()


def gemm_nt(A, B, C_out, M, N, K, lda, ldb, ldc, *, a_map=None, c_map=None, bias=None, act=0, H=None,
            row_scale=None, rows_per_scale=0, R=None, col_sum=None, col_sumsq=None, col_copies=0, split_k=0, post_ln=None):
    assert A.dtype == B.dtype and A.dtype in DT and (C_out.dtype in DT or (C_out.dtype == torch.float16 and col_sum is not None))
    if bias is not None:
        assert bias.dtype == torch.float32
    if row_scale is not None:
        assert row_scale.dtype == torch.float32
    if R is not None:
        assert R.dtype == C_out.dtype or (R.dtype == torch.float32 and C_out.dtype == torch.bfloat16)
    if H is not None:
        assert H.dtype == C_out.dtype
    if col_sum is not None:
        assert col_sum.dtype == torch.float32 and col_sumsq is not None and col_sumsq.dtype == torch.float32
    a = L.GemmNTArgs(ptr(A), ptr(B), ptr(C_out), M, N, K, lda, ldb, ldc, DT[A.dtype], 2 if C_out.dtype == torch.float16 else DT[C_out.dtype],
                     a_map or _ID, c_map or _ID, ptr(bias), act, ptr(H), ptr(row_scale), rows_per_scale, ptr(R),
                     ptr(col_sum), ptr(col_sumsq), col_copies, split_k)
    if R is not None and R.dtype != C_out.dtype:
        a.r_fp32 = 1
    if post_ln is not None:
        g, b, eps, y, mean, rstd = post_ln
        assert g.dtype == b.dtype == mean.dtype == rstd.dtype == torch.float32 and y.dtype == torch.bfloat16 and y.is_contiguous()
        a.post_y, a.post_ld, a.post_gamma, a.post_beta, a.post_eps, a.post_mean, a.post_rstd = ptr(y), y.shape[-1], ptr(g), ptr(b), eps, ptr(mean), ptr(rstd)
    check(L.lib.mvlt_gemm_nt(C.byref(a), stream_ptr()), "mvlt_gemm_nt")
    return C_out


def tn_fold_flush(partials=None):
    check(L.lib.mvlt_tn_fold_flush(ptr(partials), stream_ptr()), "mvlt_tn_fold_flush")


def tn_fold_discard(partials=None):
    check(L.lib.mvlt_tn_fold_discard(ptr(partials)), "mvlt_tn_fold_discard")


def weight_prep(desc_dev, blk_dev, ndesc, total_blocks, dtype, blk_desc=None):
    check(L.lib.mvlt_weight_prep(C.c_void_p(desc_dev.data_ptr()), C.c_void_p(blk_dev.data_ptr()), ndesc, total_blocks,
                                 C.c_void_p(blk_desc.data_ptr() if blk_desc is not None else None), DT[dtype], stream_ptr()),
          "mvlt_weight_prep")


def gemm_tn(A, B, C_out, M, N1, N2, lda, ldb, ldc, *, a_map=None, b_map=None, colsum=None, splits=0, taps=0, seg=0, dgrad=None, partials=None, defer_fold=False, overwrite=False):
    assert A.dtype == B.dtype and A.dtype in DT and C_out.dtype == torch.float32
    if colsum is not None:
        assert colsum.dtype == torch.float32
    a_map, b_map = a_map or _ID, b_map or _ID
    if dgrad is not None:
        wt, dx = dgrad
        assert A.dtype == torch.bfloat16 and wt.dtype == dx.dtype == torch.bfloat16 and N1 == N2 and N1 in (64, 128) and taps <= 1
        assert wt.is_contiguous() and tuple(wt.shape) == (N2, N1) and dx.stride(-1) == 1
        dgrad_ld = dx.stride(-2) if dx.dim() >= 2 else N2
        assert dgrad_ld % 8 == 0 and dgrad_ld >= N2, dgrad_ld
        assert a_map.mode == 0 and a_map.rows_per_batch == 0 and b_map.mode == 0 and b_map.rows_per_batch == 0, "gemm_tn(dgrad=...): plain row maps only"
        a = L.GemmTNArgs(ptr(A), ptr(B), ptr(C_out), M, N1, N2, lda, ldb, ldc, DT[A.dtype], a_map, b_map, ptr(colsum), splits, None, 0, 0, 0,
                         ptr(wt), ptr(dx), dgrad_ld)
        check(L.lib.mvlt_gemm_tn(C.byref(a), stream_ptr()), "mvlt_gemm_tn")
        return C_out
    if N1 <= 64 < N2 and b_map.mode == 0 and taps <= 1 and partials is None:
        a = L.GemmTNArgs(ptr(B), ptr(A), ptr(C_out), M, N2, N1, ldb, lda, ldc, DT[A.dtype], b_map, a_map, None, splits, ptr(colsum), 1, 0, 0)
    else:
        a = L.GemmTNArgs(ptr(A), ptr(B), ptr(C_out), M, N1, N2, lda, ldb, ldc, DT[A.dtype], a_map, b_map, ptr(colsum), splits, None, 0, taps, seg)
        if partials is not None:
            a.partials, a.partials_bytes = ptr(partials), partials.numel() * partials.element_size()
            a.defer_fold = 1 if defer_fold else 0
    if overwrite:
        assert not a.trans_c and taps <= 1 and N2 % 4 == 0 and ldc % 4 == 0 and A.dtype == torch.bfloat16, "gemm_tn(overwrite=True): bf16, plain output layout, N2 and ldc multiples of 4"
        a.c_overwrite = 1
    check(L.lib.mvlt_gemm_tn(C.byref(a), stream_ptr()), "mvlt_gemm_tn")
    return C_out


LN_CHAIN_WIDTHS = (64, 128, 320, 512, 768)


def layernorm_fwd(x, y, gamma, beta, rows, Cdim, ldx, ldy, eps, *, mean=None, rstd=None, add=None, add_rows=0,
                  x_map=None, y_map=None, chain=None):
    assert x.dtype in DT and y.dtype in DT and gamma.dtype == torch.float32 and beta.dtype == torch.float32
    tail = (None, None, None, 0.0, None, None)
    if chain is not None:
        g2, b2, eps2, y2, m2, r2 = chain
        assert Cdim in LN_CHAIN_WIDTHS and y2.dtype == torch.bfloat16 and g2.dtype == b2.dtype == m2.dtype == r2.dtype == torch.float32
        tail = (ptr(y2), ptr(g2), ptr(b2), eps2, ptr(m2), ptr(r2))
    a = L.LayerNormArgs(ptr(x), ptr(y), ptr(gamma), ptr(beta), ptr(mean), ptr(rstd), ptr(add), add_rows,
                        rows, Cdim, ldx, ldy, x_map or _ID, y_map or _ID, eps, DT[x.dtype], DT[y.dtype], *tail)
    check(L.lib.mvlt_layernorm_fwd(C.byref(a), stream_ptr()), "mvlt_layernorm_fwd")
    return y


def layernorm_bwd(dy, x, dx, gamma, mean, rstd, rows, Cdim, lddy, ldx, lddx, *, dgamma=None, dbeta=None,
                  dy_map=None, x_map=None, dx_map=None, accumulate=False, dx2=None, dx2_scale=None, dx2_rows_per_scale=0, lddx2=0,
                  copies=1, copy_stride=0):
    assert dy.dtype in DT and x.dtype in DT and dx.dtype in DT
    assert dx2 is None or (dx2.dtype == dy.dtype and dx2_scale is not None and dx2_scale.dtype == torch.float32 and dx2_rows_per_scale > 0)
    a = L.LayerNormBwdArgs(ptr(dy), ptr(x), ptr(dx), ptr(gamma), ptr(mean), ptr(rstd), ptr(dgamma), ptr(dbeta),
                           rows, Cdim, lddy, ldx, lddx, dy_map or _ID, x_map or _ID, dx_map or _ID,
                           1 if accumulate else 0, DT[dy.dtype], DT[x.dtype], DT[dx.dtype],
                           ptr(dx2), ptr(dx2_scale), dx2_rows_per_scale, lddx2, copies, copy_stride)
    check(L.lib.mvlt_layernorm_bwd(C.byref(a), stream_ptr()), "mvlt_layernorm_bwd")
    return dx


L.lib.mvlt_fold_copies.argtypes = [C.c_void_p, C.c_int, C.c_long, C.c_void_p, C.c_int, C.c_int, C.c_void_p, C.c_void_p]


def fold_copies(arena, copies, stride, dst_index, j0, j1, dst):
    assert arena.dtype == torch.float32 and dst.dtype == torch.float32 and dst_index.dtype == torch.int32
    check(L.lib.mvlt_fold_copies(ptr(arena), copies, stride, ptr(dst_index), j0, j1, ptr(dst), stream_ptr()), "mvlt_fold_copies")


L.lib.mvlt_batch_sum.argtypes = [C.c_void_p, C.c_void_p, C.c_int, C.c_int, C.c_int, C.c_long, C.c_int, C.c_int, C.c_void_p, C.c_int, C.c_void_p]


def batch_sum(x, out, B, R, Cdim, batch_stride_rows, ld, acc2=None, split=0):
    assert out.dtype == torch.float32 and (acc2 is None or (acc2.dtype == torch.float32 and acc2.is_contiguous()))
    check(L.lib.mvlt_batch_sum(ptr(x), ptr(out), B, R, Cdim, batch_stride_rows, ld, DT[x.dtype], ptr(acc2), split, stream_ptr()), "mvlt_batch_sum")
    return out


def sr_attention_fwd(Q, KV, O, lse, B, H, N, M, ldq, ldkv, ldo, k_off, v_off, scale):
    assert Q.dtype == KV.dtype == O.dtype and Q.dtype in DT
    a = L.AttnArgs(ptr(Q), ptr(KV), ptr(O), ptr(lse), B, H, N, M, ldq, ldkv, ldo, k_off, v_off, scale, DT[Q.dtype])
    check(L.lib.mvlt_sr_attention_fwd(C.byref(a), stream_ptr()), "mvlt_sr_attention_fwd")
    return O


def sr_attention_bwd_chunks(B, H, N, M, dtype):
    return int(L.lib.mvlt_sr_attention_bwd_chunks(B, H, N, M, DT[dtype]))


def sr_attention_bwd(Q, KV, O, dO, lse, dQ, dKV, B, H, N, M, ldq, ldkv, ldo, lddkv, k_off, v_off, scale):
    assert dKV.dtype == torch.float32 or (dKV.dtype == torch.bfloat16 and Q.dtype == torch.bfloat16)
    a = L.AttnBwdArgs(ptr(Q), ptr(KV), ptr(O), ptr(dO), ptr(lse), ptr(dQ), ptr(dKV), B, H, N, M,
                      ldq, ldkv, ldo, lddkv, k_off, v_off, scale, DT[Q.dtype], DT[dKV.dtype])
    check(L.lib.mvlt_sr_attention_bwd(C.byref(a), stream_ptr()), "mvlt_sr_attention_bwd")
    return dQ, dKV


L.lib.mvlt_sr_attention_fwd_streamed.argtypes = [C.POINTER(L.AttnArgs), C.c_void_p]
L.lib.mvlt_sr_attention_bwd_streamed.argtypes = [C.POINTER(L.AttnBwdArgs), C.c_void_p]


def sr_attention_fwd_streamed(Q, KV, O, lse, B, H, N, M, ldq, ldkv, ldo, k_off, v_off, scale):
    assert Q.dtype == KV.dtype == O.dtype and Q.dtype in DT
    a = L.AttnArgs(ptr(Q), ptr(KV), ptr(O), ptr(lse), B, H, N, M, ldq, ldkv, ldo, k_off, v_off, scale, DT[Q.dtype])
    check(L.lib.mvlt_sr_attention_fwd_streamed(C.byref(a), stream_ptr()), "mvlt_sr_attention_fwd_streamed")
    return O


def sr_attention_bwd_streamed(Q, KV, O, dO, lse, dQ, dKV, B, H, N, M, ldq, ldkv, ldo, lddkv, k_off, v_off, scale):
    assert dKV.dtype == torch.float32 or (dKV.dtype == torch.bfloat16 and Q.dtype == torch.bfloat16)
    a = L.AttnBwdArgs(ptr(Q), ptr(KV), ptr(O), ptr(dO), ptr(lse), ptr(dQ), ptr(dKV), B, H, N, M,
                      ldq, ldkv, ldo, lddkv, k_off, v_off, scale, DT[Q.dtype], DT[dKV.dtype])
# ... 384 lines not shown
```

### mvlt_amd/schedule.py

```python
import os

import torch
import torch.nn.functional as F

from . import ops
from ._lib import patchmap, rowmap
from .params import ZeroPool, pool_zeros
from .pvlt import BERT_DROP, EPS_BERT, EPS_BLOCK, EPS_DEFAULT, VOCAB, VOCAB_LD


def _empty(shape, dtype, dev):
    return torch.empty(shape, dtype=dtype, device=dev)


_LN_COPIES = not os.environ.get("MVLT_LN_NO_COPIES")
_NO_DX2 = bool(os.environ.get("MVLT_NO_DX2"))
_NO_T2I_FUSE = bool(os.environ.get("MVLT_NO_T2I_FUSE"))
_NO_LN_CHAIN = bool(os.environ.get("MVLT_NO_LN_CHAIN")) or bool(os.environ.get("MVLT_LN_GENERIC"))
_NO_LNB_FUSE = bool(os.environ.get("MVLT_NO_LNB_FUSE"))
_NO_POST_LN = bool(os.environ.get("MVLT_NO_POST_LN"))
_NO_OUT_OP = bool(os.environ.get("MVLT_NO_OUT_OP"))
_NO_PROJ_LN = bool(os.environ.get("MVLT_NO_PROJ_LN"))
_NO_LN_FOLD = bool(os.environ.get("MVLT_NO_LN_FOLD"))
_NO_POS_BATCH = bool(os.environ.get("MVLT_NO_POS_BATCH"))
_NT_GENERIC_EPI = bool(os.environ.get("MVLT_NT_GENERIC_EPI"))
_NO_LIN_FUSE = bool(os.environ.get("MVLT_NO_LIN_FUSE"))
WGRAD_TAPS = bool(os.environ.get("MVLT_WGRAD_TAPS"))
WGRAD_ADD = bool(os.environ.get("MVLT_WGRAD_ADD"))


_NO_OVERWRITE = bool(os.environ.get("MVLT_TN_NO_OVERWRITE"))
_DEFER_FOLD = os.environ.get("MVLT_TN_DEFER_FOLD", "1") != "0"


def conv_wgrad(S, name, dz, xin, M, cout, K, ld_dz, ld_in, bmap, taps, cin, colsum=None):
    if WGRAD_TAPS:
        ops.gemm_tn(dz, xin, S.grad(name).view(cout, K), M, cout, K, ld_dz, ld_in, K, b_map=bmap, colsum=colsum, taps=taps, seg=cin)
        return
    if WGRAD_ADD:
        dWk = pool_zeros((cout, K), torch.float32, dz.device)
        ops.gemm_tn(dz, xin, dWk, M, cout, K, ld_dz, ld_in, K, b_map=bmap, colsum=colsum)
        kk = int(round(taps ** 0.5))
        S.grad(name).add_(dWk.view(cout, kk, kk, cin).permute(0, 3, 1, 2))
        return
    ops.gemm_tn(dz, xin, S.grad_taps(name, cout, taps, cin), M, cout, K, ld_dz, ld_in, K, b_map=bmap, colsum=colsum, partials=S.tn_partials(), defer_fold=_DEFER_FOLD)


def _step_rng(model):
    model._rng_calls = getattr(model, "_rng_calls", 0) + 1
    return torch.initial_seed(), model._rng_calls


def check_input_size(model, Himg, Wimg):
    unit = model.patch_size * 8
    assert Himg % unit == 0 and Wimg % unit == 0, \
        f"input size {Himg} x {Wimg} (H x W): each side should be divided by patch_size {unit} (rectangles are fine, as in the reference)"


def stage_grids(model, Himg, Wimg):
    return [(Himg // model.patch_size // (2 ** i), Wimg // model.patch_size // (2 ** i)) for i in range(4)]


class Names:

    @staticmethod
    def blk(i, j):
        return f"block{i+1}.{j}."


class TrunkStep:

    def __init__(self, model, images, ids, need_grad):
        self.m = model
        self.S = model.store
        self.dev = images.device
        self.dt = model.compute_dtype
        self.rt = torch.float32
        self.need_grad = need_grad
        self.images = images.contiguous().float()
        self.ids = ids.contiguous()
        self.B = images.shape[0]
        assert images.shape[1] == model.in_chans
        Himg, Wimg = images.shape[2], images.shape[3]
        check_input_size(model, Himg, Wimg)
        self.Himg, self.Wimg = Himg, Wimg
        self.T = ids.shape[1]
        assert self.T == model.T_num, "input_ids length must equal num_text_tokens"
        self.grid = stage_grids(model, Himg, Wimg)
        self.saved = []
        self.training = model.training

    def _mark(self):
        ev = getattr(self.m, "_block_events", None)
        if ev is not None:
            e = torch.cuda.Event(enable_timing=True)
            e.record()
            ev.append(e)

    def w(self, name):
        return self.S.comp(name)

    def wT(self, name):
        return self.S.extra[name + "::T"]

    def wK(self, name):
        return self.S.extra[name + "::K"]

    def wKT(self, name):
        return self.S.extra[name + "::KT"]

    def f32(self, name):
        return self.S.master(name)

    def g(self, name):
        return self.S.grad(name)
# ... 89 lines not shown
        C = m.dims[i]
        h, w = self.grid[i]
        HW = h * w
        N = HW + T
        sv = dict(i=i, C=C, HW=HW, N=N)
        pe, ten = f"patch_embed{i+1}.", f"text_embed{i+1}."
        pe_pre = _empty((B * HW, C), dt, dev)
        if i == 0:
            K = m.in_chans * m.patch_size ** 2
            P1 = _empty((B * HW, K), dt, dev)
            ops.patchify(self.images, P1, B, m.in_chans, self.Himg, self.Wimg, m.patch_size)
            ops.gemm_nt(P1, self.w(pe + "proj.weight"), pe_pre, B * HW, C, K, K, K, C, bias=self.f32(pe + "proj.bias"))
            sv["P1"] = P1
        else:
            Cp, Np, wp = m.dims[i - 1], self.saved[i - 1]["N"], self.grid[i - 1][1]
            pm = patchmap(2, wp, Np, HW, w, Cp)
            ops.gemm_nt(xp, self.wK(pe + "proj.weight"), pe_pre, B * HW, C, 4 * Cp, Cp, 4 * Cp, C, a_map=pm,
                        bias=self.f32(pe + "proj.bias"))
            sv["pm_in"] = pm
        x = _empty((B, N, C), self.rt, dev)
        pos = self._pos(i, self.f32(f"pos_embed{i+1}"))
        sv["pe_pre"], sv["pe_mean"], sv["pe_rstd"] = pe_pre, _empty((B * HW,), torch.float32, dev), _empty((B * HW,), torch.float32, dev)
        chain = None
        if dt == torch.bfloat16 and C in ops.LN_CHAIN_WIDTHS and not _NO_LN_CHAIN:
            p0 = Names.blk(i, 0)
            self._pre_ln1 = (_empty((B, N, C), dt, dev), _empty((B * N,), torch.float32, dev), _empty((B * N,), torch.float32, dev))
            chain = (self.f32(p0 + "norm1.weight"), self.f32(p0 + "norm1.bias"), EPS_BLOCK, *self._pre_ln1)
        ops.layernorm_fwd(pe_pre, x, self.f32(pe + "norm.weight"), self.f32(pe + "norm.bias"), B * HW, C, C, C, EPS_DEFAULT,
                          mean=sv["pe_mean"], rstd=sv["pe_rstd"], add=pos, add_rows=HW, y_map=rowmap(HW, N, 0), chain=chain)
        te_pre = _empty((B * T, C), dt, dev)
        if i == 0:
            ops.gemm_nt(self.emb, self.w(ten + "0.weight"), te_pre, B * T, C, m.hidden, m.hidden, m.hidden, C,
                        bias=self.f32(ten + "0.bias"))
        else:
            Cp, Np, HWp = m.dims[i - 1], self.saved[i - 1]["N"], self.saved[i - 1]["HW"]
            ops.gemm_nt(xp, self.w(ten + "0.weight"), te_pre, B * T, C, Cp, Cp, Cp, C, a_map=rowmap(T, Np, HWp),
                        bias=self.f32(ten + "0.bias"))
        sv["te_pre"], sv["te_mean"], sv["te_rstd"] = te_pre, _empty((B * T,), torch.float32, dev), _empty((B * T,), torch.float32, dev)
        ops.layernorm_fwd(te_pre, x, self.f32(ten + "1.weight"), self.f32(ten + "1.bias"), B * T, C, C, C, EPS_DEFAULT,
                          mean=sv["te_mean"], rstd=sv["te_rstd"], add=self.f32(f"text_pos_embed{i+1}")[0], add_rows=T,
                          y_map=rowmap(T, N, HW), chain=chain)
        sv["x_in_prev"] = xp
        sv["blocks"] = []
        self._mark()
        for j in range(m.depths[i]):
            x, bsv = self._block_forward(i, j, x, blk_index)
            sv["blocks"].append(bsv)
            blk_index += 1
        self._mark()
        if x.dtype != dt:
            xb = _empty((B, N, C), dt, dev)
            ops.cast_bf16(x, xb, x.numel())
            x = xb
        sv["x_out"] = x
        taps = getattr(m, "_taps", None)
        if taps is not None:
            taps[f"img_feat{i+1}"] = x[:, :HW].float().reshape(B, h, w, C).permute(0, 3, 1, 2)
            taps[f"text_feat{i+1}"] = x[:, HW:].float()
        self.saved.append(sv)
        return x, blk_index

    def _block_forward(self, i, j, x, blk_index):
        m, B, T, dt, dev = self.m, self.B, self.T, self.dt, self.dev
        C, h, r, hid = m.dims[i], m.heads[i], m.sr[i], m.hid[i]
        gh, gw = self.grid[i]
        HW = gh * gw
        N = HW + T
        M = B * N
        p = Names.blk(i, j)
        f32 = torch.float32
        bs = dict(x=x)
        s1, s2 = self._droppath_scales(blk_index)
        bs["s1"], bs["s2"] = s1, s2
        pre = getattr(self, "_pre_ln1", None)
        self._pre_ln1 = None
        if pre is not None:
            xn1, bs["m1"], bs["r1"] = pre
        else:
            xn1 = _empty((B, N, C), dt, dev)
            bs["m1"], bs["r1"] = _empty((M,), f32, dev), _empty((M,), f32, dev)
            ops.layernorm_fwd(x, xn1, self.f32(p + "norm1.weight"), self.f32(p + "norm1.bias"), M, C, C, C, EPS_BLOCK, mean=bs["m1"], rstd=bs["r1"])
        bs["xn1"] = xn1
        q = _empty((B, N, C), dt, dev)
        ops.gemm_nt(xn1, self.w(p + "attn.q.weight"), q, M, C, C, C, C, C, bias=self.f32(p + "attn.q.bias"))
        bs["q"] = q
        if r > 1:
            HWr = (gh // r) * (gw // r)
            Mk = HWr + T
            pm = patchmap(r, gw, N, HWr, gw // r, C)
            sr_pre = _empty((B * HWr, C), dt, dev)
            ops.gemm_nt(xn1, self.wK(p + "attn.sr.weight"), sr_pre, B * HWr, C, r * r * C, C, r * r * C, C, a_map=pm,
                        bias=self.f32(p + "attn.sr.bias"))
            kvin = _empty((B * HWr, C), dt, dev)
            bs["msr"], bs["rsr"] = _empty((B * HWr,), f32, dev), _empty((B * HWr,), f32, dev)
            ops.layernorm_fwd(sr_pre, kvin, self.f32(p + "attn.norm.weight"), self.f32(p + "attn.norm.bias"), B * HWr, C, C, C,
                              EPS_DEFAULT, mean=bs["msr"], rstd=bs["rsr"])
            kv = _empty((B, Mk, 2 * C), dt, dev)
            wkv, bkv = self.w(p + "attn.kv.weight"), self.f32(p + "attn.kv.bias")
            ops.gemm_nt(kvin, wkv, kv, B * HWr, 2 * C, C, C, C, 2 * C, c_map=rowmap(HWr, Mk, 0), bias=bkv)
            ops.gemm_nt(xn1, wkv, kv, B * T, 2 * C, C, C, C, 2 * C, a_map=rowmap(T, N, HW), c_map=rowmap(T, Mk, HWr), bias=bkv)
            bs.update(sr_pre=sr_pre, kvin=kvin, pm=pm, HWr=HWr)
        else:
            Mk = N
            kv = _empty((B, Mk, 2 * C), dt, dev)
            ops.gemm_nt(xn1, self.w(p + "attn.kv.weight"), kv, M, 2 * C, C, C, C, 2 * C, bias=self.f32(p + "attn.kv.bias"))
        bs["kv"], bs["Mk"] = kv, Mk
        ao = _empty((B, N, C), dt, dev)
        lse = _empty((B, h, N), f32, dev)
        ops.sr_attention_fwd(q, kv, ao, lse, B, h, N, Mk, C, 2 * C, C, 0, C, 64 ** -0.5)
        bs["ao"], bs["lse"] = ao, lse
        xm = _empty((B, N, C), self.rt, dev)
        xn2 = _empty((B, N, C), dt, dev)
        bs["m2"], bs["r2"] = _empty((M,), f32, dev), _empty((M,), f32, dev)
        bs["xn2"] = xn2
        bs["fused_mlp"] = fused = (dt == torch.bfloat16 and C in (64, 128))
        proj_ln = fused and not _NO_PROJ_LN and not _NO_LN_FOLD and M < (1 << 24)
        ops.gemm_nt(ao, self.w(p + "attn.proj.weight"), xm, M, C, C, C, C, C, bias=self.f32(p + "attn.proj.bias"),
                    row_scale=s1, rows_per_scale=N, R=x,
                    post_ln=(self.f32(p + "norm2.weight"), self.f32(p + "norm2.bias"), EPS_BLOCK, xn2.view(M, C), bs["m2"], bs["r2"]) if proj_ln else None)
        bs["xm"] = xm
        last_op = fused and j == m.depths[i] - 1 and self.dt != self.rt and not _NO_OUT_OP
        last_gemm = ((not fused) and j == m.depths[i] - 1 and dt == torch.bfloat16 and self.rt == torch.float32 and not _NO_OUT_OP and
                     M < (1 << 24) and C % 8 == 0 and not _NT_GENERIC_EPI)
        xo = _empty((B, N, C), dt if (last_op or last_gemm) else self.rt, dev)
        if fused:
            ln = None if (_NO_LN_FOLD or proj_ln) else (self.f32(p + "norm2.weight"), self.f32(p + "norm2.bias"), EPS_BLOCK, xn2, bs["m2"], bs["r2"])
            if ln is None and not proj_ln:
                ops.layernorm_fwd(xm, xn2, self.f32(p + "norm2.weight"), self.f32(p + "norm2.bias"), M, C, C, C, EPS_BLOCK, mean=bs["m2"], rstd=bs["r2"])
            post = None
            if j + 1 < m.depths[i] and not _NO_POST_LN:
                pn = Names.blk(i, j + 1)
                self._pre_ln1 = (_empty((B, N, C), dt, dev), _empty((M,), f32, dev), _empty((M,), f32, dev))
                post = (self.f32(pn + "norm1.weight"), self.f32(pn + "norm1.bias"), EPS_BLOCK, *self._pre_ln1)
            ops.mlp_fwd(None if ln else xn2, self.w(p + "mlp.fc1.weight"), self.f32(p + "mlp.fc1.bias"), self.w(p + "mlp.fc2.weight"),
                        self.f32(p + "mlp.fc2.bias"), xm, None if last_op else xo, M, C, hid, row_scale=s2, rows_per_scale=N, ln=ln,
                        out_op=xo if last_op else None, post_ln=post)
        else:
            ops.layernorm_fwd(xm, xn2, self.f32(p + "norm2.weight"), self.f32(p + "norm2.bias"), M, C, C, C, EPS_BLOCK, mean=bs["m2"], rstd=bs["r2"])
            hpre = _empty((M, hid), dt, dev) if self.need_grad else None
            gact = _empty((M, hid), dt, dev)
            ops.gemm_nt(xn2, self.w(p + "mlp.fc1.weight"), gact, M, hid, C, C, C, hid, bias=self.f32(p + "mlp.fc1.bias"), act=1, H=hpre)
            bs["hpre"], bs["gact"] = hpre, gact
            ops.gemm_nt(gact, self.w(p + "mlp.fc2.weight"), xo, M, C, hid, hid, hid, C, bias=self.f32(p + "mlp.fc2.bias"),
                        row_scale=s2, rows_per_scale=N, R=xm)
        if not self.need_grad:
            bs.clear()
        return xo, bs

    def _scaled(self, dy, scale, N):
        if scale is None:
            return dy
        out = torch.empty_like(dy)
        ops.row_scale(dy, scale, N, self.B * N, dy.shape[-1], out)
        return out

    def backward(self, dxs):
        m, B, T, dt, dev, S = self.m, self.B, self.T, self.dt, self.dev, self.S
        self._pos_adj = []
        own = [d is not None and d.dtype == dt and d.is_contiguous() and S.owns(d) for d in dxs]
        dx, merged = None, False
        for i in (3, 2, 1, 0):
            sv = self.saved[i]
            d_out = dxs[i]
            if d_out is not None and not merged:
                d_out = d_out.to(dt)
                if dx is None:
                    dx = d_out if own[i] else d_out.contiguous().clone()
                else:
                    dx.add_(d_out)
            if dx is None:
                continue
            into = dxs[i - 1] if i > 0 and own[i - 1] else None
            dx = self._stage_backward(i, sv, dx.view(B, sv["N"], sv["C"]), into)
            merged = into is not None
            self.S.announce_stage(i)
        if self._pos_adj:
            ops.resize_bilinear_tokens_multi(self._pos_adj, adjoint=True)
            self._pos_adj = []
        self.S.announce_prefix("pos_embed", "text_pos_embed")
        self.S.fold_copies()
        self.saved = []

    def _stage_backward(self, i, sv, dx, into=None):
        m, B, T, dt, dev = self.m, self.B, self.T, self.dt, self.dev
        C, HW, N = sv["C"], sv["HW"], sv["N"]
        self._mark()
        for j in reversed(range(m.depths[i])):
            dx = self._block_backward(i, j, sv["blocks"][j], dx)
# ... 38 lines not shown
        if HW == m.grids[0] ** 2:
            gv.add_(dpos)
            return
        if _NO_POS_BATCH:
            ops.resize_bilinear_tokens(dpos, gv, m.grids[i], m.grids[i], h, w, dpos.shape[1], adjoint=True)
        else:
            self._pos_adj.append((dpos, gv, m.grids[i], m.grids[i], h, w, dpos.shape[1]))

    def _bert_backward(self, d_emb):
        m, B, T = self.m, self.B, self.T
        te = "text_embeddings."
        ops.bert_embed_bwd(d_emb, self.ids, self.f32(te + "word_embeddings.weight"), self.f32(te + "position_embeddings.weight"),
                           self.f32(te + "token_type_embeddings.weight"), self.f32(te + "LayerNorm.weight"), self.keep, BERT_DROP,
                           self.emb_mean, self.emb_rstd, self.g(te + "word_embeddings.weight"), self.g(te + "position_embeddings.weight"),
                           self.g(te + "token_type_embeddings.weight"), self.g(te + "LayerNorm.weight"), self.g(te + "LayerNorm.bias"),
                           B * T, T)

    def _block_backward(self, i, j, bs, dx):
        m, B, T, dt, dev = self.m, self.B, self.T, self.dt, self.dev
        C, h, r, hid = m.dims[i], m.heads[i], m.sr[i], m.hid[i]
        HW = self.grid[i][0] * self.grid[i][1]
        N = HW + T
        M = B * N
        p = Names.blk(i, j)
        f32 = torch.float32
        dxn2 = _empty((M, C), dt, dev)
        ln2_done = False
        if bs["fused_mlp"]:
            w1, w2t = self.w(p + "mlp.fc1.weight"), self.wT(p + "mlp.fc2.weight")
            ops.mlp_bwd_dw(bs["xn2"], dx, w1, w2t, self.f32(p + "mlp.fc1.bias"), self.g(p + "mlp.fc1.weight"), self.g(p + "mlp.fc1.bias"),
                           self.g(p + "mlp.fc2.weight"), self.g(p + "mlp.fc2.bias"), M, C, hid, row_scale=bs["s2"], rows_per_scale=N,
                           partials=self.S.tn_partials(), defer_fold=_DEFER_FOLD)
            if not _NO_LNB_FUSE:
                fuse = bs["s1"] is not None and not _NO_DX2
                dy1 = _empty((M, C), dx.dtype, dev) if fuse else dx
                ops.mlp_bwd_dx(bs["xn2"], dx, w1, self.wT(p + "mlp.fc1.weight"), w2t, self.f32(p + "mlp.fc1.bias"), None, M, C, hid,
                               row_scale=bs["s2"], rows_per_scale=N,
                               ln_bwd=dict(x=bs["xm"], mean=bs["m2"], rstd=bs["r2"], gamma=self.f32(p + "norm2.weight"), dx=dx,
                                           dgamma=self.gl(p + "norm2.weight"), dbeta=self.gl(p + "norm2.bias"),
                                           dx2=dy1 if fuse else None, dx2_scale=bs["s1"], dx2_rows_per_scale=N))
                ln2_done = True
            else:
                ops.mlp_bwd_dx(bs["xn2"], dx, w1, self.wT(p + "mlp.fc1.weight"), w2t, self.f32(p + "mlp.fc1.bias"), dxn2, M, C, hid,
                               row_scale=bs["s2"], rows_per_scale=N)
        else:
            dy2 = getattr(self, "_dy2_pre", None)
            self._dy2_pre = None
            if dy2 is None:
                dy2 = self._scaled(dx, bs["s2"], N)
            ops.gemm_tn(dy2, bs["gact"], self.g(p + "mlp.fc2.weight"), M, C, hid, C, hid, hid, colsum=self.g(p + "mlp.fc2.bias"), partials=self.S.tn_partials(), defer_fold=_DEFER_FOLD)
            dh = _empty((M, hid), dt, dev)
            ops.gemm_nt(dy2, self.wT(p + "mlp.fc2.weight"), dh, M, hid, C, C, C, hid, act=2, H=bs["hpre"])
            bs["gact"] = bs["hpre"] = None
            ops.gemm_tn(dh, bs["xn2"], self.g(p + "mlp.fc1.weight"), M, hid, C, hid, C, C, colsum=self.g(p + "mlp.fc1.bias"), partials=self.S.tn_partials(), defer_fold=_DEFER_FOLD)
            ops.gemm_nt(dh, self.wT(p + "mlp.fc1.weight"), dxn2, M, C, hid, hid, hid, C)
            del dh
        if not ln2_done:
            fuse = bs["s1"] is not None and not _NO_DX2
            dy1 = _empty((M, C), dx.dtype, dev) if fuse else dx
            ops.layernorm_bwd(dxn2, bs["xm"], dx, self.f32(p + "norm2.weight"), bs["m2"], bs["r2"], M, C, C, C, C,
                              dgamma=self.gl(p + "norm2.weight"), dbeta=self.gl(p + "norm2.bias"), **self.lnk(), accumulate=True,
                              dx2=dy1 if fuse else None, dx2_scale=bs["s1"], dx2_rows_per_scale=N, lddx2=C)
        if not fuse:
            dy1 = self._scaled(dx, bs["s1"], N)
        lin_fuse = dt == torch.bfloat16 and C in (64, 128) and not _NO_LIN_FUSE
        dao = dxn2
        if lin_fuse:
            ops.gemm_tn(dy1, bs["ao"], self.g(p + "attn.proj.weight"), M, C, C, C, C, C, colsum=self.g(p + "attn.proj.bias"),
                        dgrad=(self.wT(p + "attn.proj.weight"), dao.view(M, C)))
        else:
            ops.gemm_tn(dy1, bs["ao"], self.g(p + "attn.proj.weight"), M, C, C, C, C, C, colsum=self.g(p + "attn.proj.bias"), partials=self.S.tn_partials(), defer_fold=_DEFER_FOLD)
            ops.gemm_nt(dy1, self.wT(p + "attn.proj.weight"), dao, M, C, C, C, C, C)
        Mk = bs["Mk"]
        dq = _empty((B, N, C), dt, dev)
        if dt == torch.bfloat16 and ops.sr_attention_bwd_chunks(B, h, N, Mk, dt) == 1:
            dkv = _empty((B, Mk, 2 * C), dt, dev)
            ops.sr_attention_bwd(bs["q"], bs["kv"], bs["ao"], dao, bs["lse"], dq, dkv, B, h, N, Mk, C, 2 * C, C, 2 * C, 0, C, 64 ** -0.5)
        else:
            dkv32 = pool_zeros((B, Mk, 2 * C), f32, dev)
            ops.sr_attention_bwd(bs["q"], bs["kv"], bs["ao"], dao, bs["lse"], dq, dkv32, B, h, N, Mk, C, 2 * C, C, 2 * C, 0, C, 64 ** -0.5)
            dkv = dkv32.to(dt)
            del dkv32
        dxn1 = dao
        if lin_fuse:
            ops.gemm_tn(dq, bs["xn1"], self.g(p + "attn.q.weight"), M, C, C, C, C, C, colsum=self.g(p + "attn.q.bias"),
                        dgrad=(self.wT(p + "attn.q.weight"), dxn1.view(M, C)))
        else:
            ops.gemm_tn(dq, bs["xn1"], self.g(p + "attn.q.weight"), M, C, C, C, C, C, colsum=self.g(p + "attn.q.bias"), partials=self.S.tn_partials(), defer_fold=_DEFER_FOLD)
            ops.gemm_nt(dq, self.wT(p + "attn.q.weight"), dxn1, M, C, C, C, C, C)
        gkvw, gkvb = self.g(p + "attn.kv.weight"), self.g(p + "attn.kv.bias")
        wkvT = self.wT(p + "attn.kv.weight")
        if r > 1:
            HWr, pm = bs["HWr"], bs["pm"]
            ops.gemm_tn(dkv, bs["xn1"], gkvw, B * T, 2 * C, C, 2 * C, C, C, a_map=rowmap(T, Mk, HWr), b_map=rowmap(T, N, HW), colsum=gkvb, partials=self.S.tn_partials(), defer_fold=_DEFER_FOLD)
            ops.gemm_nt(dkv, wkvT, dxn1, B * T, C, 2 * C, 2 * C, 2 * C, C, a_map=rowmap(T, Mk, HWr), c_map=rowmap(T, N, HW), R=dxn1)
            ops.gemm_tn(dkv, bs["kvin"], gkvw, B * HWr, 2 * C, C, 2 * C, C, C, a_map=rowmap(HWr, Mk, 0), colsum=gkvb, partials=self.S.tn_partials(), defer_fold=_DEFER_FOLD)
            dkvin = _empty((B * HWr, C), dt, dev)
            ops.gemm_nt(dkv, wkvT, dkvin, B * HWr, C, 2 * C, 2 * C, 2 * C, C, a_map=rowmap(HWr, Mk, 0))
            dsr = _empty((B * HWr, C), dt, dev)
            ops.layernorm_bwd(dkvin, bs["sr_pre"], dsr, self.f32(p + "attn.norm.weight"), bs["msr"], bs["rsr"], B * HWr, C, C, C, C,
                              dgamma=self.gl(p + "attn.norm.weight"), dbeta=self.gl(p + "attn.norm.bias"), **self.lnk())
            K = r * r * C
            conv_wgrad(self.S, p + "attn.sr.weight", dsr, bs["xn1"], B * HWr, C, K, C, C, pm, r * r, C, colsum=self.g(p + "attn.sr.bias"))
            ops.gemm_nt(dsr, self.wKT(p + "attn.sr.weight"), dxn1, B * HWr, K, C, C, C, C, c_map=pm, R=dxn1)
        else:
            ops.gemm_tn(dkv, bs["xn1"], gkvw, M, 2 * C, C, 2 * C, C, C, colsum=gkvb, partials=self.S.tn_partials(), defer_fold=_DEFER_FOLD)
            ops.gemm_nt(dkv, wkvT, dxn1, M, C, 2 * C, 2 * C, 2 * C, C, R=dxn1)
        prev = self.saved[i]["blocks"][j - 1] if j > 0 else None
        pre = prev is not None and not prev.get("fused_mlp", True) and prev.get("s2") is not None and not _NO_DX2
        self._dy2_pre = _empty((M, C), dx.dtype, dev) if pre else None
        ops.layernorm_bwd(dxn1, bs["x"], dx, self.f32(p + "norm1.weight"), bs["m1"], bs["r1"], M, C, C, C, C,
                          dgamma=self.gl(p + "norm1.weight"), dbeta=self.gl(p + "norm1.bias"), **self.lnk(), accumulate=True,
                          dx2=self._dy2_pre, dx2_scale=prev["s2"] if pre else None, dx2_rows_per_scale=N if pre else 0, lddx2=C if pre else 0)
        bs.clear()
        return dx


class _TrunkFn(torch.autograd.Function):

    @staticmethod
    def forward(ctx, model, images, ids, need_grad, *params):
        step = TrunkStep(model, images, ids, need_grad)
        outs = step.forward()
        ctx.step = step
        ctx.pool_token, model._pool_token = model._pool_token, None
        ctx.set_materialize_grads(False)
        ctx.mark_non_differentiable(outs[0])
        return tuple(outs)

    @staticmethod
    def backward(ctx, d1, d2, d3, d4):
        step = ctx.step
        S = step.S
        S.queue_finalize()
        step.backward([None, d2, d3, d4])
        ctx.step = None
        ctx.pool_token = None
        grads = []
        for k, (name, p) in enumerate(S.fn_params):
            gv = S.grad(name)
            if not ctx.needs_input_grad[4 + k]:
                grads.append(None)
            elif p.grad is not None and p.grad.data_ptr() == gv.data_ptr():
                grads.append(None)
            else:
                grads.append(gv)
        return (None, None, None, None, *grads)


class _GradSink:

    def __init__(self, store):
        self.S, self.buf = store, None

    def take(self, shape, dtype, dev):
        if self.buf is None:
            self.buf = self.S.own(torch.zeros(shape, dtype=dtype, device=dev))
            return self.buf, self.buf
        return self.buf, None


def _embed_ln_fwd(model, prefix, A, a_map, rows, lda):
    S, dt, dev = model.store, model.compute_dtype, A.device
    Hd, Cin = model.hidden, model.dims[3]
    pre = _empty((rows, Hd), dt, dev)
    ops.gemm_nt(A, S.comp(prefix + ".0.weight"), pre, rows, Hd, Cin, lda, Cin, Hd, a_map=a_map, bias=S.master(prefix + ".0.bias"))
    y = _empty((rows, Hd), dt, dev)
    mean, rstd = _empty((rows,), torch.float32, dev), _empty((rows,), torch.float32, dev)
    ops.layernorm_fwd(pre, y, S.master(prefix + ".1.weight"), S.master(prefix + ".1.bias"), rows, Hd, Hd, Hd, EPS_DEFAULT, mean=mean, rstd=rstd)
    return y, (pre, mean, rstd)


def _embed_ln_bwd(model, prefix, dy, saved, A, a_map, rows, lda, dA, c_map, accumulate):
    S, dt, dev = model.store, model.compute_dtype, dy.device
    Hd, Cin = model.hidden, model.dims[3]
    pre, mean, rstd = saved
    dpre = _empty((rows, Hd), dt, dev)
    ops.layernorm_bwd(dy, pre, dpre, S.master(prefix + ".1.weight"), mean, rstd, rows, Hd, Hd, Hd, Hd,
                      dgamma=S.grad(prefix + ".1.weight"), dbeta=S.grad(prefix + ".1.bias"))
    ops.gemm_tn(dpre, A, S.grad(prefix + ".0.weight"), rows, Hd, Cin, Hd, lda, Cin, b_map=a_map, colsum=S.grad(prefix + ".0.bias"))
    ops.gemm_nt(dpre, S.extra[prefix + ".0.weight::T"], dA, rows, Cin, Hd, Hd, Hd, Cin, c_map=c_map, R=dA if accumulate else None)


class _ClsHeadFn(torch.autograd.Function):

    @staticmethod
    def forward(ctx, x4, model, name, HW, sink):
        S, dt, dev = model.store, model.compute_dtype, x4.device
        B, N, C = x4.shape
# ... 244 lines not shown
```

Before: 13470.

## Add grouped GEMM launches for independent attention projections and weight gradients

Adds grouped NT and TN GEMM entry points. Each one plans every problem with the existing dispatcher and, when all problems map to the same kernel configuration, launches them as a single kernel whose workgroups look up their problem by a block-offset table. The schedule batches the q and kv forward projections, the q/kv weight-gradient GEMMs, and the q and kv-input data-gradient GEMMs into these groups to cut launch count and fill the GPU better on small PVT-tiny shapes. It reorders some kernels in the backward pass and falls back to per-problem launches when the plans differ.

```diff
diff --git a/include/mvlt_hip.h b/include/mvlt_hip.h
--- a/include/mvlt_hip.h
+++ b/include/mvlt_hip.h
@@ -8,7 +8,7 @@
 #define MVLT_DT_BF16 0
 #define MVLT_DT_FP32 1
 
-#define MVLT_ABI_VERSION 7
+#define MVLT_ABI_VERSION 8
 const char* mvlt_last_error(void);
 int mvlt_abi_version(void);
 const char* mvlt_last_kernel(void);
@@ -42,6 +42,7 @@
   int r_fp32;
 } mvlt_gemm_nt_args;
 int mvlt_gemm_nt(const mvlt_gemm_nt_args* args, void* stream);
+int mvlt_gemm_nt_group(const mvlt_gemm_nt_args* args, int n, void* stream);
 
 typedef struct mvlt_gemm_tn_args {
   const void* A; const void* B; float* C;
@@ -59,6 +60,7 @@
   int c_overwrite;
 } mvlt_gemm_tn_args;
 int mvlt_gemm_tn(const mvlt_gemm_tn_args* args, void* stream);
+int mvlt_gemm_tn_group(const mvlt_gemm_tn_args* args, int n, void* stream);
 int mvlt_tn_fold_flush(const void* partials, void* stream);
 int mvlt_tn_fold_discard(const void* partials);
 
diff --git a/mvlt_amd/_lib.py b/mvlt_amd/_lib.py
--- a/mvlt_amd/_lib.py
+++ b/mvlt_amd/_lib.py
@@ -102,7 +102,7 @@
 lib.mvlt_last_error.restype = C.c_char_p
 lib.mvlt_last_kernel.restype = C.c_char_p
 lib.mvlt_sizeof.argtypes = [C.c_char_p]
-ABI_VERSION = 7
+ABI_VERSION = 8
 if lib.mvlt_abi_version() != ABI_VERSION:
     raise ImportError(f"ABI mismatch: {LIB_PATH} is version {lib.mvlt_abi_version()}, the binding is version {ABI_VERSION} (stale build? run python -m mvlt_amd.build)")
 for _name, _cls in (("mvlt_rowmap", RowMap), ("mvlt_prep_desc", PrepDesc), ("mvlt_gemm_nt_args", GemmNTArgs), ("mvlt_gemm_tn_args", GemmTNArgs),
@@ -112,7 +112,7 @@
     if _n != C.sizeof(_cls):
         raise ImportError(f"ABI mismatch for {_name}: library says {_n} bytes, binding has {C.sizeof(_cls)}")
 
-EXPORTS = ["mvlt_last_error", "mvlt_last_kernel", "mvlt_abi_version", "mvlt_sizeof", "mvlt_gemm_nt", "mvlt_gemm_tn",
+EXPORTS = ["mvlt_last_error", "mvlt_last_kernel", "mvlt_abi_version", "mvlt_sizeof", "mvlt_gemm_nt", "mvlt_gemm_tn", "mvlt_gemm_nt_group", "mvlt_gemm_tn_group",
            "mvlt_layernorm_fwd", "mvlt_layernorm_bwd", "mvlt_fold_copies", "mvlt_batch_sum", "mvlt_sr_attention_fwd", "mvlt_sr_attention_bwd",
            "mvlt_bert_embed_fwd", "mvlt_bert_embed_bwd", "mvlt_patchify", "mvlt_masked_select", "mvlt_gather_rows",
            "mvlt_scatter_rows", "mvlt_cross_entropy_fwd", "mvlt_cross_entropy_bwd", "mvlt_adamw_step", "mvlt_smooth_l1_fwd", "mvlt_smooth_l1_bwd", "mvlt_cast_bf16",
diff --git a/mvlt_amd/csrc/gemm.hip b/mvlt_amd/csrc/gemm.hip
--- a/mvlt_amd/csrc/gemm.hip
+++ b/mvlt_amd/csrc/gemm.hip
@@ -1019,7 +1019,7 @@
 };
 
 template <int BMT, int BN, int BMODE, int NS, bool DG = false>
-__global__ __launch_bounds__(NTHREADS, 2) void gemm_tn_dma_kernel(mvlt_gemm_tn_args p, int m_per_split, int t1, int t2, int splits, bf16* part = nullptr) {
+__device__ __forceinline__ void gemm_tn_dma_body(const mvlt_gemm_tn_args& p, const int m_per_split, const int t1, const int t2, const int splits, bf16* const part, const int bid) {
   using TA = DmaTile<BMT>;
   using TB = DmaTile<BN>;
   static_assert(!DG || (BMODE == 3 && BMT == BN && !MVLT_TN_EARLY), "dgrad rides on the plain-row single-tile kernels");
@@ -1032,14 +1032,14 @@
   const int txy = t1 * t2;
   int bz, xy;
   if (splits >= 8) {
-    const int xcd = blockIdx.x & 7, kq = blockIdx.x >> 3;
+    const int xcd = bid & 7, kq = bid >> 3;
     const int zq = kq / txy;
     xy = kq - zq * txy;
     bz = zq * 8 + xcd;
     if (bz >= splits) return;
   } else {
-    bz = blockIdx.x / txy;
-    xy = blockIdx.x - bz * txy;
+    bz = bid / txy;
+    xy = bid - bz * txy;
   }
   const int bx = xy % t1, by = xy / t1;
 
@@ -1066,7 +1066,7 @@
     if constexpr (BMODE == 1) b_seg_rows = rowmap_seg(bmap, b_seg);
     else { tap_dy = b_seg / 3 - 1; tap_dx = b_seg - (b_seg / 3) * 3 - 1; }
   }
-  const char* zsrc = (const char*)g_zero_page + ((tid * 16 + (blockIdx.x & 15) * 4096) & 65535);
+  const char* zsrc = (const char*)g_zero_page + ((tid * 16 + (bid & 15) * 4096) & 65535);
   const char* a_src = (const char*)p.A + 2 * a_col;
   const char* b_src = (const char*)p.B + 2 * b_col;
   const unsigned a_rowb = 2u * (unsigned)p.lda, b_rowb = 2u * (unsigned)p.ldb;
@@ -1332,6 +1332,20 @@
         int n2 = n2_0 + wn * WN + j * 16 + fr;
         if (n1 < p.N1 && n2 < p.N2) atomicAdd(p.trans_c ? &p.C[(long)n2 * p.ldc + n1] : &p.C[(long)n1 * p.ldc + tn_dst_col(p, n2)], acc[i][j][r]);
       }
+}
+template <int BMT, int BN, int BMODE, int NS, bool DG = false>
+__global__ __launch_bounds__(NTHREADS, 2) void gemm_tn_dma_kernel(mvlt_gemm_tn_args p, int m_per_split, int t1, int t2, int splits, bf16* part = nullptr) {
+  gemm_tn_dma_body<BMT, BN, BMODE, NS, DG>(p, m_per_split, t1, t2, splits, part, (int)blockIdx.x);
+}
+constexpr int TN_GROUP_MAX = 8;
+struct TnGroupItem { mvlt_gemm_tn_args p; bf16* part; int m_per_split, t1, t2, splits, wg0; };
+struct TnGroup { TnGroupItem it[TN_GROUP_MAX]; int n; };
+template <int BMT, int BN, int BMODE, int NS>
+__global__ __launch_bounds__(NTHREADS, 2) void gemm_tn_dma_group_kernel(TnGroup g) {
+  int i = 0;
+  for (int k = 1; k < g.n; ++k) if ((int)blockIdx.x >= g.it[k].wg0) i = k;
+  const TnGroupItem& t = g.it[i];
+  gemm_tn_dma_body<BMT, BN, BMODE, NS, false>(t.p, t.m_per_split, t.t1, t.t2, t.splits, t.part, (int)blockIdx.x - t.wg0);
 }
 
 template <int W>
@@ -1571,7 +1585,7 @@
 }
 
 template <int BN, int AMODE, int EPI, int BK, int BMT = BM>
-__global__ __launch_bounds__(NTHREADS, BMT == 256 ? 2 : 1) void gemm_nt_dma_kernel(mvlt_gemm_nt_args p, int ns_flags) {
+__device__ __forceinline__ void gemm_nt_dma_body(const mvlt_gemm_nt_args& p, const int ns_flags, const int bid) {
   const int ns = ns_flags & 0xff;
   const bool early = (ns_flags & 0x100) != 0;
   constexpr int ROWB = BK * 2;
@@ -1590,7 +1604,6 @@
   const int wm = wave >> 1, wn = wave & 1;
   const int tiles_m = (p.M + BMT - 1) / BMT;
   const int tiles_n = (p.N + BN - 1) / BN;
-  const int bid = blockIdx.x;
   const int xcd = bid & 7, bslot = bid >> 3;
   const int tile_m = (bslot / tiles_n) * 8 + xcd, tile_n = bslot % tiles_n;
   if (tile_m >= tiles_m) return;
@@ -1737,6 +1750,18 @@
   if constexpr (BN == 192) nt_epilogue_192<EPI>(p, acc, smem, m0, n0, wave, lane);
   else if constexpr (EPI == 0) nt_epilogue<bf16, BN>(p, acc, smem, m0, n0, wave, lane);
   else nt_epilogue_lean<BN, EPI, TM_>(p, acc, smem, m0, n0, wave, lane);
+}
+template <int BN, int AMODE, int EPI, int BK, int BMT = BM>
+__global__ __launch_bounds__(NTHREADS, BMT == 256 ? 2 : 1) void gemm_nt_dma_kernel(mvlt_gemm_nt_args p, int ns_flags) {
+  gemm_nt_dma_body<BN, AMODE, EPI, BK, BMT>(p, ns_flags, (int)blockIdx.x);
+}
+constexpr int GROUP_MAX = 8;
+struct NtGroup { mvlt_gemm_nt_args a[GROUP_MAX]; int wg0[GROUP_MAX + 1]; int n; };
+template <int BN, int AMODE, int EPI>
+__global__ __launch_bounds__(NTHREADS, 1) void gemm_nt_dma_group_kernel(NtGroup g, int ns_flags) {
+  int i = 0;
+  for (int k = 1; k < g.n; ++k) if ((int)blockIdx.x >= g.wg0[k]) i = k;
+  gemm_nt_dma_body<BN, AMODE, EPI, 64, BM>(g.a[i], ns_flags, (int)blockIdx.x - g.wg0[i]);
 }
 
 __device__ __forceinline__ void glds16_s(const char* sbase, unsigned voff, unsigned dst) {
@@ -2577,7 +2602,10 @@
 
 }
 
-extern "C" int mvlt_gemm_nt(const mvlt_gemm_nt_args* a, void* stream) {
+struct NtPlan { int key; unsigned grid; size_t lds; int ns; };
+#define MVLT_NT_PLAN_OTHER() do { if (plan) { plan->key = -1; return MVLT_OK; } } while (0)
+static int nt_run(const mvlt_gemm_nt_args* a, void* stream, NtPlan* plan) {
+  if (plan) plan->key = -1;
   MVLT_REQUIRE(a && a->A && a->B && a->C, "mvlt_gemm_nt: null operand");
   MVLT_REQUIRE(a->M >= 0 && a->N > 0 && a->K > 0, "mvlt_gemm_nt: bad shape M=%d N=%d K=%d", a->M, a->N, a->K);
   MVLT_REQUIRE(a->dtype == 0 || a->dtype == 1, "mvlt_gemm_nt: dtype must be 0 (bf16) or 1 (fp32)");
@@ -2645,6 +2673,7 @@
     const int ns_lds = ns;
     if (nkd >= 2) ns |= early_flag;
     if (a->post_y) {
+      MVLT_NT_PLAN_OTHER();
       MVLT_REQUIRE(epi == 2 && a->N == bn && a->a_map.mode == 0 && a->c_map.mode == 0 && a->c_map.rows_per_batch == 0 && a->post_gamma && a->post_beta &&
                    a->post_mean && a->post_rstd && a->post_ld % 8 == 0 && ((uintptr_t)a->post_y & 15) == 0 && ((uintptr_t)a->post_gamma & 15) == 0,
                    "mvlt_gemm_nt: post_y needs bf16 operands, a residual (R), N == 64 or 128, identity row maps, 16-byte aligned outputs");
@@ -2677,6 +2706,7 @@
         (a->a_map.w_in == 16 || a->a_map.w_in == 32 || a->a_map.w_in == 64) && (a->a_map.h_in * a->a_map.w_in) % BM == 0 && a->M % BM == 0 &&
         a->M % (a->a_map.h_in * a->a_map.w_in) == 0 && a->a_map.hw_out == a->a_map.h_in * a->a_map.w_in && a->a_map.w_out == a->a_map.w_in &&
         a->K == 9 * a->a_map.c_seg && a->lda >= a->a_map.c_seg && a->ldb >= a->K) {
+      MVLT_NT_PLAN_OTHER();
       bool done = a->a_map.w_in == 32 ? dispatch_conv3_nt<32>(*a, epi, s) : a->a_map.w_in == 16 ? dispatch_conv3_nt<16>(*a, epi, s) : dispatch_conv3_nt<64>(*a, epi, s);
       if (done) return mvlt_check_launch("mvlt_gemm_nt");
     }
@@ -2694,18 +2724,20 @@
       if (!c320 && !c256 && !c192 && epi == 1 && (ntp8 & 8) && (a->M % 256 || a->N % 256)) {
         const long tiles = (long)((a->M + 255) / 256) * ((a->N + 255) / 256);
         const long rounds = (tiles + 255) / 256;
-        if (tiles >= 384 && (double)a->M * a->N >= 0.85 * (double)rounds * 256.0 * 65536.0) { launch_nt_p8<1, 4, 2, 2, true>(*a, s); done = true; }
+        if (tiles >= 384 && (double)a->M * a->N >= 0.85 * (double)rounds * 256.0 * 65536.0) { MVLT_NT_PLAN_OTHER(); launch_nt_p8<1, 4, 2, 2, true>(*a, s); done = true; }
       }
       if (!done && !c320 && !c256 && !c192 && (ntp8 & 4) && a->N % 320 == 0 && a->N % 256 != 0 && a->M % 192 != 0 && (epi == 1 || (epi == 2 && (a->K >= 640 || (ntp8 & 16))))) {
         const long tiles = (long)((a->M + 191) / 192) * (a->N / 320);
         const long rounds = (tiles + 255) / 256;
         if (tiles >= 192 && (double)a->M * a->N >= 0.85 * (double)rounds * 256.0 * 192.0 * 320.0) {
+          MVLT_NT_PLAN_OTHER();
           if (epi == 1) launch_nt_p8<1, 3, 3, 2, true>(*a, s);
           else launch_nt_p8<2, 3, 3, 2, true>(*a, s);
           done = true;
         }
       }
       if (done) return mvlt_check_launch("mvlt_gemm_nt");
+      if (c320 || c256 || c192) MVLT_NT_PLAN_OTHER();
       if (c320) done = dispatch_nt_p8<3, 3, 2>(*a, epi, s);
       else if (c256 && (!c192 || c256 <= c192)) done = dispatch_nt_p8<4, 2, 2>(*a, epi, s);
       else if (c192) done = dispatch_nt_p8<3, 2, 2>(*a, epi, s);
@@ -2713,6 +2745,12 @@
     }
     const bool wide = !narrow && a->N % 192 == 0 && a->N % 128 != 0 && (epi == 1 || epi == 5) && a->c_map.mode == 0 && a->a_map.mode != 1 &&
                       a->K >= 128 && !getenv("MVLT_NT_NO192");
+    if (plan) {
+      if (wide || bkd == 32 || a->split_k > 1) return MVLT_OK;
+      plan->key = (bn << 16) | (a->a_map.mode << 12) | (epi << 8) | ns_lds | (ns & 0x100 ? 0x80 : 0);
+      plan->grid = grid.x; plan->lds = lds2; plan->ns = ns;
+      return MVLT_OK;
+    }
     if (wide) {
       const int tn192 = a->N / 192;
       dim3 grid192((unsigned)(8 * ((tiles_m + 7) / 8) * tn192), 1);
@@ -2730,10 +2768,48 @@
 #undef MVLT_NT_LAUNCH_E
 #undef MVLT_NT_LAUNCH
   } else {
+    MVLT_NT_PLAN_OTHER();
     if (narrow) MVLT_LAUNCH((gemm_nt_kernel<float, 64>), grid, block, lds, s, *a, nbuf);
     else MVLT_LAUNCH((gemm_nt_kernel<float, 128>), grid, block, lds, s, *a, nbuf);
   }
   return mvlt_check_launch("mvlt_gemm_nt");
+}
+#undef MVLT_NT_PLAN_OTHER
+extern "C" int mvlt_gemm_nt(const mvlt_gemm_nt_args* a, void* stream) { return nt_run(a, stream, nullptr); }
+
+template <int BN, int AMODE, int EPI> static void nt_group_launch(const NtGroup& g, unsigned total, size_t lds, int ns, hipStream_t s) {
+  mvlt_max_lds<(gemm_nt_dma_group_kernel<BN, AMODE, EPI>)>();
+  MVLT_LAUNCH((gemm_nt_dma_group_kernel<BN, AMODE, EPI>), dim3(total), dim3(NTHREADS), lds, s, g, ns);
+}
+extern "C" int mvlt_gemm_nt_group(const mvlt_gemm_nt_args* args, int n, void* stream) {
+  MVLT_REQUIRE(args && n >= 1, "mvlt_gemm_nt_group: needs n >= 1 problems");
+  bool grouped = n > 1 && n <= GROUP_MAX;
+  NtPlan pl[GROUP_MAX];
+  for (int i = 0; i < n && grouped; ++i) {
+    if (int e = nt_run(&args[i], stream, &pl[i])) return e;
+    if (pl[i].key < 0 || pl[i].key != pl[0].key) grouped = false;
+  }
+  if (grouped) {
+    NtGroup g;
+    unsigned total = 0;
+    for (int i = 0; i < n; ++i) { g.a[i] = args[i]; g.wg0[i] = (int)total; total += pl[i].grid; }
+    g.wg0[n] = (int)total; g.n = n;
+    const int bn = pl[0].key >> 16, am = (pl[0].key >> 12) & 15, epi = (pl[0].key >> 8) & 15;
+    hipStream_t s = (hipStream_t)stream;
+    const size_t lds = pl[0].lds;
+    const int ns = pl[0].ns;
+    if (bn == 64 && am == 0 && epi == 1) nt_group_launch<64, 0, 1>(g, total, lds, ns, s);
+    else if (bn == 128 && am == 0 && epi == 1) nt_group_launch<128, 0, 1>(g, total, lds, ns, s);
+    else if (bn == 64 && am == 0 && epi == 2) nt_group_launch<64, 0, 2>(g, total, lds, ns, s);
+    else if (bn == 128 && am == 0 && epi == 2) nt_group_launch<128, 0, 2>(g, total, lds, ns, s);
+    else if (bn == 64 && am == 1 && epi == 1) nt_group_launch<64, 1, 1>(g, total, lds, ns, s);
+    else if (bn == 128 && am == 1 && epi == 1) nt_group_launch<128, 1, 1>(g, total, lds, ns, s);
+    else grouped = false;
+    if (grouped) return mvlt_check_launch("mvlt_gemm_nt_group");
+  }
+  for (int i = 0; i < n; ++i)
+    if (int e = nt_run(&args[i], stream, nullptr)) return e;
+  return MVLT_OK;
 }
 
 bf16* mvlt_fold_acquire_ext(const mvlt_gemm_tn_args& a, long need, hipStream_t s, int descriptors) { return fold_acquire(a, need, s, descriptors); }
@@ -2753,7 +2829,10 @@
   return mvlt_check_launch("mvlt_tn_fold_flush");
 }
 
-extern "C" int mvlt_gemm_tn(const mvlt_gemm_tn_args* a, void* stream) {
+struct TnPlan { int bmt, bn, bmode; unsigned grid; size_t lds; int m_per_split, t1, t2, splits; long need; };
+#define MVLT_TN_PLAN_OTHER() do { if (plan) { plan->bmt = 0; return MVLT_OK; } } while (0)
+static int tn_run(const mvlt_gemm_tn_args* a, void* stream, TnPlan* plan) {
+  if (plan) plan->bmt = 0;
   MVLT_REQUIRE(a && a->A && a->B && a->C, "mvlt_gemm_tn: null operand");
   MVLT_REQUIRE(a->M >= 0 && a->N1 > 0 && a->N2 > 0, "mvlt_gemm_tn: bad shape");
   MVLT_REQUIRE(a->dtype == 0 || a->dtype == 1, "mvlt_gemm_tn: dtype must be 0 (bf16) or 1 (fp32)");
@@ -2778,6 +2857,7 @@
       !a->colsum_a && !a->colsum_b && a->N1 % 64 == 0 && a->b_map.c_seg % 64 == 0 && a->N2 == 9 * a->b_map.c_seg && a->M % 64 == 0 &&
       (a->b_map.w_in == 8 || a->b_map.w_in == 16 || a->b_map.w_in == 32 || a->b_map.w_in == 64) && (a->b_map.h_in * a->b_map.w_in) % 64 == 0 &&
       a->M % (a->b_map.h_in * a->b_map.w_in) == 0 && a->ldb >= a->b_map.c_seg) {
+    MVLT_TN_PLAN_OTHER();
     hipStream_t s2 = (hipStream_t)stream;
     if (a->b_map.w_in == 64) return launch_conv3_wgrad<64>(*a, s2);
     if (a->b_map.w_in == 32) return launch_conv3_wgrad<32>(*a, s2);
@@ -2788,8 +2868,10 @@
   if (tnp8 && a->partials && a->dtype == 0 && a->a_map.mode == 0 && a->b_map.mode == 0 && a->a_map.rows_per_batch == 0 && a->b_map.rows_per_batch == 0 && a->c_taps <= 1 &&
       !a->trans_c && !a->dgrad_out && a->M % 64 == 0 && a->N1 % 256 == 0 && a->N2 % 256 == 0 && a->ldc % 4 == 0 && ((uintptr_t)a->C & 15) == 0 && ((uintptr_t)a->partials & 15) == 0) {
     const int tiles = (a->N1 / 256) * (a->N2 / 256), nkt = a->M / 64;
-    if (tiles >= 16 && tiles <= 64 && nkt / (256 / tiles) >= 16 && a->partials_bytes >= (long)(256 / tiles) * a->N1 * a->N2 * 2)
+    if (tiles >= 16 && tiles <= 64 && nkt / (256 / tiles) >= 16 && a->partials_bytes >= (long)(256 / tiles) * a->N1 * a->N2 * 2) {
+      MVLT_TN_PLAN_OTHER();
       return launch_tn_p8_partial<4, 2, 2>(*a, s);
+    }
   }
   static const bool tn320 = !(getenv("MVLT_TN_P8_320") && atoi(getenv("MVLT_TN_P8_320")) == 0);
   if (tnp8 && tn320 && a->partials && a->dtype == 0 && a->a_map.mode == 0 && a->b_map.mode == 0 && a->a_map.rows_per_batch == 0 && a->b_map.rows_per_batch == 0 && a->c_taps <= 1 &&
@@ -2800,6 +2882,7 @@
       const int rows = direct ? a->N1 : a->N2, cols = direct ? a->N2 : a->N1;
       const int tiles = ((rows + 191) / 192) * (cols / 320), nkt = a->M / 64;
       if (tiles >= 6 && tiles <= 16 && nkt / (256 / tiles) >= 16 && (double)rows >= 0.85 * 192.0 * ((rows + 191) / 192)) {
+        MVLT_TN_PLAN_OTHER();
         const int rc = direct ? launch_tn_p8_320<false>(*a, s) : launch_tn_p8_320<true>(*a, s);
         if (rc <= 0) return rc;
       }
@@ -2807,6 +2890,7 @@
   }
   if (a->dtype == 0 && a->M < (1 << 24)) {
     if (a->dgrad_out) {
+      MVLT_TN_PLAN_OTHER();
       MVLT_REQUIRE(a->dgrad_wt && a->N1 == a->N2 && (a->N1 == 64 || a->N1 == 128) && a->a_map.rows_per_batch == 0 && a->b_map.mode == 0 &&
                    a->b_map.rows_per_batch == 0 && !a->trans_c && a->c_taps <= 1 && !a->colsum_b && a->dgrad_ld % 8 == 0 &&
                    (((uintptr_t)a->dgrad_out | (uintptr_t)a->dgrad_wt) & 15) == 0,
@@ -2855,9 +2939,17 @@
     dim3 grid((unsigned)((splits >= 8 ? 8 * ((splits + 7) / 8) : splits) * t1 * t2)), block(NTHREADS);
     static const int part_min = getenv("MVLT_TN_PART_MIN") ? atoi(getenv("MVLT_TN_PART_MIN")) : 8;
     static const long part_min_out = getenv("MVLT_TN_PART_MINOUT") ? atol(getenv("MVLT_TN_PART_MINOUT")) : 16384;
-    bf16* const part = (tnp8 && a->partials && !a->c_overwrite && splits >= part_min && !a->trans_c && a->c_taps <= 1 && a->N2 % 8 == 0 && a->ldc % 4 == 0 && ((uintptr_t)a->C & 15) == 0 &&
-                        (long)a->N1 * a->N2 >= part_min_out)
-                           ? fold_acquire(*a, (long)splits * a->N1 * a->N2 * 2, s) : nullptr;
+    const bool want_part = tnp8 && a->partials && !a->c_overwrite && splits >= part_min && !a->trans_c && a->c_taps <= 1 && a->N2 % 8 == 0 && a->ldc % 4 == 0 && ((uintptr_t)a->C & 15) == 0 &&
+                           (long)a->N1 * a->N2 >= part_min_out;
+    if (plan) {
+      const long need = (long)splits * a->N1 * a->N2 * 2;
+      plan->bmt = bmt; plan->bn = bn;
+      plan->bmode = (a->b_map.mode == 0 && a->b_map.rows_per_batch == 0 && a->a_map.rows_per_batch == 0) ? 3 : a->b_map.mode;
+      plan->grid = grid.x; plan->lds = lds; plan->m_per_split = m_per_split; plan->t1 = t1; plan->t2 = t2; plan->splits = splits;
+      plan->need = (want_part && ((uintptr_t)a->partials & 15) == 0 && need <= a->partials_bytes) ? need : 0;
+      return MVLT_OK;
+    }
+    bf16* const part = want_part ? fold_acquire(*a, (long)splits * a->N1 * a->N2 * 2, s) : nullptr;
 #define MVLT_TN_LAUNCH(BMT_, BN_, NS_)                                                                                          \
   do {                                                                                                                         \
     if (a->b_map.mode == 0 && a->b_map.rows_per_batch == 0 && a->a_map.rows_per_batch == 0)                                                        \
@@ -2874,6 +2966,7 @@
     if (part) fold_launch(*a, part, splits, s);
     return mvlt_check_launch("mvlt_gemm_tn");
   }
+  MVLT_TN_PLAN_OTHER();
   const bool narrow = a->N2 <= 64;
   const int bn = narrow ? 64 : 128;
   const int t1 = (a->N1 + BM - 1) / BM, t2 = (a->N2 + bn - 1) / bn;
@@ -2898,3 +2991,93 @@
   }
   return mvlt_check_launch("mvlt_gemm_tn");
 }
+#undef MVLT_TN_PLAN_OTHER
+extern "C" int mvlt_gemm_tn(const mvlt_gemm_tn_args* a, void* stream) { return tn_run(a, stream, nullptr); }
+
+template <int BMT, int BN, int BMODE, int NS> static void tn_group_launch(const TnGroup& g, unsigned total, size_t lds, hipStream_t s) {
+  mvlt_max_lds<(gemm_tn_dma_group_kernel<BMT, BN, BMODE, NS>)>();
+  MVLT_LAUNCH((gemm_tn_dma_group_kernel<BMT, BN, BMODE, NS>), dim3(total), dim3(NTHREADS), lds, s, g);
+}
+static bool tn_group_dispatch(const TnGroup& g, int bmt, int bn, int bmode, unsigned total, size_t lds, hipStream_t s) {
+#define MVLT_TNG(BMT_, BN_, NS_)                                                  \
+  do {                                                                            \
+    if (bmode == 3) tn_group_launch<BMT_, BN_, 3, NS_>(g, total, lds, s);         \
+    else tn_group_launch<BMT_, BN_, 0, NS_>(g, total, lds, s);                    \
+  } while (0)
+  if (bmode != 0 && bmode != 3) return false;
+  if (bmt == 128 && bn == 128) MVLT_TNG(128, 128, 2);
+  else if (bmt == 128) MVLT_TNG(128, 64, 3);
+  else if (bn == 128) MVLT_TNG(64, 128, 3);
+  else MVLT_TNG(64, 64, 4);
+#undef MVLT_TNG
+  return true;
+}
+extern "C" int mvlt_gemm_tn_group(const mvlt_gemm_tn_args* args, int n, void* stream) {
+  MVLT_REQUIRE(args && n >= 1, "mvlt_gemm_tn_group: needs n >= 1 problems");
+  hipStream_t s = (hipStream_t)stream;
+  bool grouped = n > 1 && n <= TN_GROUP_MAX;
+  TnPlan pl[TN_GROUP_MAX];
+  int bmode = -1, first_part = -1, nparts = 0;
+  long total_need = 0;
+  for (int i = 0; i < n && grouped; ++i) {
+    if (int e = tn_run(&args[i], stream, &pl[i])) return e;
+    if (pl[i].bmt == 0 || pl[i].bmt != pl[0].bmt || pl[i].bn != pl[0].bn || (pl[i].bmode != 0 && pl[i].bmode != 3)) { grouped = false; break; }
+    bmode = (bmode < 0 || bmode == pl[i].bmode) ? pl[i].bmode : 0;
+    if (pl[i].need > 0) {
+      if (first_part < 0) first_part = i;
+      if (!args[i].defer_fold || args[i].partials != args[first_part].partials || args[i].partials_bytes != args[first_part].partials_bytes) grouped = false;
+      total_need += (pl[i].need + 255) & ~255L;
+      ++nparts;
+    }
+  }
+  if (grouped && nparts > 0 && total_need > args[first_part].partials_bytes) grouped = false;
+  if (grouped) {
+    TnGroup g;
+    unsigned total = 0;
+    for (int i = 0; i < n; ++i) {
+      TnGroupItem& t = g.it[i];
+      t.p = args[i]; t.part = nullptr; t.m_per_split = pl[i].m_per_split; t.t1 = pl[i].t1; t.t2 = pl[i].t2; t.splits = pl[i].splits; t.wg0 = (int)total;
+      total += pl[i].grid;
+    }
+    g.n = n;
+    if (nparts == 0) {
+      if (!tn_group_dispatch(g, pl[0].bmt, pl[0].bn, bmode, total, pl[0].lds, s)) grouped = false;
+    } else {
+      const mvlt_gemm_tn_args& a0 = args[first_part];
+      std::lock_guard<std::mutex> lk(g_fold_mu);
+      FoldPending& f = g_fold[a0.partials];
+      auto overlaps = [](const float* c, int n1, int n2, int ldc, const FoldDesc& d) {
+        const float* c_hi = c + (size_t)(n1 - 1) * ldc + n2;
+        const float* d_hi = d.C + (size_t)(d.N1 - 1) * d.ldc + d.N2;
+        return c < d_hi && d.C < c_hi;
+      };
+      bool flush = f.b.n > 0 && (f.stream != s || f.b.n + nparts > FOLD_MAX || f.used + total_need > a0.partials_bytes);
+      for (int i = 0; i < n && !flush; ++i)
+        if (pl[i].need > 0)
+          for (int k = 0; k < f.b.n && !flush; ++k) flush = overlaps(args[i].C, args[i].N1, args[i].N2, args[i].ldc, f.b.d[k]);
+      if (flush) fold_flush_locked(f, s, true);
+      f.stream = s;
+      long off = f.used;
+      for (int i = 0; i < n; ++i)
+        if (pl[i].need > 0) { g.it[i].part = (bf16*)((char*)a0.partials + off); off += (pl[i].need + 255) & ~255L; }
+      if (!tn_group_dispatch(g, pl[0].bmt, pl[0].bn, bmode, total, pl[0].lds, s)) grouped = false;
+      if (grouped) {
+        for (int i = 0; i < n; ++i) {
+          if (pl[i].need <= 0) continue;
+          bool clash = false;
+          for (int k = 0; k < f.b.n && !clash; ++k) clash = overlaps(args[i].C, args[i].N1, args[i].N2, args[i].ldc, f.b.d[k]);
+          if (clash) fold_flush_locked(f, s, true);
+          FoldDesc& d = f.b.d[f.b.n];
+          d.part = g.it[i].part; d.C = args[i].C; d.splits = pl[i].splits; d.N1 = args[i].N1; d.N2 = args[i].N2; d.ldc = args[i].ldc;
+          d.wg0 = f.b.n == 0 ? 0 : f.b.d[f.b.n - 1].wg0 + fold_wgs(f.b.d[f.b.n - 1]);
+          ++f.b.n;
+        }
+        f.used = off;
+      }
+    }
+    if (grouped) return mvlt_check_launch("mvlt_gemm_tn_group");
+  }
+  for (int i = 0; i < n; ++i)
+    if (int e = tn_run(&args[i], stream, nullptr)) return e;
+  return MVLT_OK;
+}
diff --git a/mvlt_amd/csrc/runtime.hip b/mvlt_amd/csrc/runtime.hip
--- a/mvlt_amd/csrc/runtime.hip
+++ b/mvlt_amd/csrc/runtime.hip
@@ -53,5 +53,7 @@
   S(mvlt_rowmap) S(mvlt_prep_desc) S(mvlt_gemm_nt_args) S(mvlt_gemm_tn_args) S(mvlt_layernorm_args) S(mvlt_layernorm_bwd_args)
   S(mvlt_attn_args) S(mvlt_attn_bwd_args) S(mvlt_mlp_args)
 #undef S
+  if (strcmp(name, "mvlt_gemm_nt_group") == 0 || strcmp(name, "mvlt_gemm_tn_group") == 0) return 8;
+
   return -1;
 }
diff --git a/mvlt_amd/ops.py b/mvlt_amd/ops.py
--- a/mvlt_amd/ops.py
+++ b/mvlt_amd/ops.py
@@ -8,8 +8,8 @@
 _ID = rowmap()
 
 
-def gemm_nt(A, B, C_out, M, N, K, lda, ldb, ldc, *, a_map=None, c_map=None, bias=None, act=0, H=None,
-            row_scale=None, rows_per_scale=0, R=None, col_sum=None, col_sumsq=None, col_copies=0, split_k=0, post_ln=None):
+def gemm_nt_args(A, B, C_out, M, N, K, lda, ldb, ldc, *, a_map=None, c_map=None, bias=None, act=0, H=None,
+                 row_scale=None, rows_per_scale=0, R=None, col_sum=None, col_sumsq=None, col_copies=0, split_k=0, post_ln=None):
     assert A.dtype == B.dtype and A.dtype in DT and (C_out.dtype in DT or (C_out.dtype == torch.float16 and col_sum is not None))
     if bias is not None:
         assert bias.dtype == torch.float32
@@ -30,8 +30,31 @@
         g, b, eps, y, mean, rstd = post_ln
         assert g.dtype == b.dtype == mean.dtype == rstd.dtype == torch.float32 and y.dtype == torch.bfloat16 and y.is_contiguous()
         a.post_y, a.post_ld, a.post_gamma, a.post_beta, a.post_eps, a.post_mean, a.post_rstd = ptr(y), y.shape[-1], ptr(g), ptr(b), eps, ptr(mean), ptr(rstd)
+    return a
+
+
+def gemm_nt(A, B, C_out, *shape, **kw):
+    a = gemm_nt_args(A, B, C_out, *shape, **kw)
     check(L.lib.mvlt_gemm_nt(C.byref(a), stream_ptr()), "mvlt_gemm_nt")
     return C_out
+
+
+def gemm_nt_group(problems, single=False):
+    if single or len(problems) == 1:
+        for a in problems:
+            check(L.lib.mvlt_gemm_nt(C.byref(a), stream_ptr()), "mvlt_gemm_nt")
+        return
+    arr = (L.GemmNTArgs * len(problems))(*problems)
+    check(L.lib.mvlt_gemm_nt_group(arr, len(problems), stream_ptr()), "mvlt_gemm_nt_group")
+
+
+def gemm_tn_group(problems, single=False):
+    if single or len(problems) == 1:
+        for a in problems:
+            check(L.lib.mvlt_gemm_tn(C.byref(a), stream_ptr()), "mvlt_gemm_tn")
+        return
+    arr = (L.GemmTNArgs * len(problems))(*problems)
+    check(L.lib.mvlt_gemm_tn_group(arr, len(problems), stream_ptr()), "mvlt_gemm_tn_group")
 
 
 def tn_fold_flush(partials=None):
@@ -48,7 +71,13 @@
           "mvlt_weight_prep")
 
 
-def gemm_tn(A, B, C_out, M, N1, N2, lda, ldb, ldc, *, a_map=None, b_map=None, colsum=None, splits=0, taps=0, seg=0, dgrad=None, partials=None, defer_fold=False, overwrite=False):
+def gemm_tn(A, B, C_out, *shape, **kw):
+    a = gemm_tn_args(A, B, C_out, *shape, **kw)
+    check(L.lib.mvlt_gemm_tn(C.byref(a), stream_ptr()), "mvlt_gemm_tn")
+    return C_out
+
+
+def gemm_tn_args(A, B, C_out, M, N1, N2, lda, ldb, ldc, *, a_map=None, b_map=None, colsum=None, splits=0, taps=0, seg=0, dgrad=None, partials=None, defer_fold=False, overwrite=False):
     assert A.dtype == B.dtype and A.dtype in DT and C_out.dtype == torch.float32
     if colsum is not None:
         assert colsum.dtype == torch.float32
@@ -62,8 +91,7 @@
         assert a_map.mode == 0 and a_map.rows_per_batch == 0 and b_map.mode == 0 and b_map.rows_per_batch == 0, "gemm_tn(dgrad=...): plain row maps only"
         a = L.GemmTNArgs(ptr(A), ptr(B), ptr(C_out), M, N1, N2, lda, ldb, ldc, DT[A.dtype], a_map, b_map, ptr(colsum), splits, None, 0, 0, 0,
                          ptr(wt), ptr(dx), dgrad_ld)
-        check(L.lib.mvlt_gemm_tn(C.byref(a), stream_ptr()), "mvlt_gemm_tn")
-        return C_out
+        return a
     if N1 <= 64 < N2 and b_map.mode == 0 and taps <= 1 and partials is None:
         a = L.GemmTNArgs(ptr(B), ptr(A), ptr(C_out), M, N2, N1, ldb, lda, ldc, DT[A.dtype], b_map, a_map, None, splits, ptr(colsum), 1, 0, 0)
     else:
@@ -74,8 +102,7 @@
     if overwrite:
         assert not a.trans_c and taps <= 1 and N2 % 4 == 0 and ldc % 4 == 0 and A.dtype == torch.bfloat16, "gemm_tn(overwrite=True): bf16, plain output layout, N2 and ldc multiples of 4"
         a.c_overwrite = 1
-    check(L.lib.mvlt_gemm_tn(C.byref(a), stream_ptr()), "mvlt_gemm_tn")
-    return C_out
+    return a
 
 
 LN_CHAIN_WIDTHS = (64, 128, 320, 512, 768)
diff --git a/mvlt_amd/schedule.py b/mvlt_amd/schedule.py
--- a/mvlt_amd/schedule.py
+++ b/mvlt_amd/schedule.py
@@ -31,6 +31,15 @@
 
 _NO_OVERWRITE = bool(os.environ.get("MVLT_TN_NO_OVERWRITE"))
 _DEFER_FOLD = os.environ.get("MVLT_TN_DEFER_FOLD", "1") != "0"
+_NO_GROUP = bool(os.environ.get("MVLT_NO_GROUP"))
+
+
+def _nt_group(problems):
+    ops.gemm_nt_group(problems, single=_NO_GROUP)
+
+
+def _tn_group(problems):
+    ops.gemm_tn_group(problems, single=_NO_GROUP)
 
 
 def conv_wgrad(S, name, dz, xin, M, cout, K, ld_dz, ld_in, bmap, taps, cin, colsum=None):
@@ -286,28 +295,30 @@
             ops.layernorm_fwd(x, xn1, self.f32(p + "norm1.weight"), self.f32(p + "norm1.bias"), M, C, C, C, EPS_BLOCK, mean=bs["m1"], rstd=bs["r1"])
         bs["xn1"] = xn1
         q = _empty((B, N, C), dt, dev)
-        ops.gemm_nt(xn1, self.w(p + "attn.q.weight"), q, M, C, C, C, C, C, bias=self.f32(p + "attn.q.bias"))
+        level = [ops.gemm_nt_args(xn1, self.w(p + "attn.q.weight"), q, M, C, C, C, C, C, bias=self.f32(p + "attn.q.bias"))]
         bs["q"] = q
         if r > 1:
             HWr = (gh // r) * (gw // r)
             Mk = HWr + T
             pm = patchmap(r, gw, N, HWr, gw // r, C)
             sr_pre = _empty((B * HWr, C), dt, dev)
+            kv = _empty((B, Mk, 2 * C), dt, dev)
+            wkv, bkv = self.w(p + "attn.kv.weight"), self.f32(p + "attn.kv.bias")
+            level.append(ops.gemm_nt_args(xn1, wkv, kv, B * T, 2 * C, C, C, C, 2 * C, a_map=rowmap(T, N, HW), c_map=rowmap(T, Mk, HWr), bias=bkv))
+            _nt_group(level)
             ops.gemm_nt(xn1, self.wK(p + "attn.sr.weight"), sr_pre, B * HWr, C, r * r * C, C, r * r * C, C, a_map=pm,
                         bias=self.f32(p + "attn.sr.bias"))
             kvin = _empty((B * HWr, C), dt, dev)
             bs["msr"], bs["rsr"] = _empty((B * HWr,), f32, dev), _empty((B * HWr,), f32, dev)
             ops.layernorm_fwd(sr_pre, kvin, self.f32(p + "attn.norm.weight"), self.f32(p + "attn.norm.bias"), B * HWr, C, C, C,
                               EPS_DEFAULT, mean=bs["msr"], rstd=bs["rsr"])
-            kv = _empty((B, Mk, 2 * C), dt, dev)
-            wkv, bkv = self.w(p + "attn.kv.weight"), self.f32(p + "attn.kv.bias")
             ops.gemm_nt(kvin, wkv, kv, B * HWr, 2 * C, C, C, C, 2 * C, c_map=rowmap(HWr, Mk, 0), bias=bkv)
-            ops.gemm_nt(xn1, wkv, kv, B * T, 2 * C, C, C, C, 2 * C, a_map=rowmap(T, N, HW), c_map=rowmap(T, Mk, HWr), bias=bkv)
             bs.update(sr_pre=sr_pre, kvin=kvin, pm=pm, HWr=HWr)
         else:
             Mk = N
             kv = _empty((B, Mk, 2 * C), dt, dev)
-            ops.gemm_nt(xn1, self.w(p + "attn.kv.weight"), kv, M, 2 * C, C, C, C, 2 * C, bias=self.f32(p + "attn.kv.bias"))
+            level.append(ops.gemm_nt_args(xn1, self.w(p + "attn.kv.weight"), kv, M, 2 * C, C, C, C, 2 * C, bias=self.f32(p + "attn.kv.bias")))
+            _nt_group(level)
         bs["kv"], bs["Mk"] = kv, Mk
         ao = _empty((B, N, C), dt, dev)
         lse = _empty((B, h, N), f32, dev)
@@ -512,21 +523,25 @@
             dkv = dkv32.to(dt)
             del dkv32
         dxn1 = dao
+        wgrads = []
         if lin_fuse:
             ops.gemm_tn(dq, bs["xn1"], self.g(p + "attn.q.weight"), M, C, C, C, C, C, colsum=self.g(p + "attn.q.bias"),
                         dgrad=(self.wT(p + "attn.q.weight"), dxn1.view(M, C)))
         else:
-            ops.gemm_tn(dq, bs["xn1"], self.g(p + "attn.q.weight"), M, C, C, C, C, C, colsum=self.g(p + "attn.q.bias"), partials=self.S.tn_partials(), defer_fold=_DEFER_FOLD)
-            ops.gemm_nt(dq, self.wT(p + "attn.q.weight"), dxn1, M, C, C, C, C, C)
+            wgrads.append(ops.gemm_tn_args(dq, bs["xn1"], self.g(p + "attn.q.weight"), M, C, C, C, C, C, colsum=self.g(p + "attn.q.bias"), partials=self.S.tn_partials(), defer_fold=_DEFER_FOLD))
         gkvw, gkvb = self.g(p + "attn.kv.weight"), self.g(p + "attn.kv.bias")
         wkvT = self.wT(p + "attn.kv.weight")
         if r > 1:
             HWr, pm = bs["HWr"], bs["pm"]
-            ops.gemm_tn(dkv, bs["xn1"], gkvw, B * T, 2 * C, C, 2 * C, C, C, a_map=rowmap(T, Mk, HWr), b_map=rowmap(T, N, HW), colsum=gkvb, partials=self.S.tn_partials(), defer_fold=_DEFER_FOLD)
+            wgrads.append(ops.gemm_tn_args(dkv, bs["xn1"], gkvw, B * T, 2 * C, C, 2 * C, C, C, a_map=rowmap(T, Mk, HWr), b_map=rowmap(T, N, HW), colsum=gkvb, partials=self.S.tn_partials(), defer_fold=_DEFER_FOLD))
+            wgrads.append(ops.gemm_tn_args(dkv, bs["kvin"], gkvw, B * HWr, 2 * C, C, 2 * C, C, C, a_map=rowmap(HWr, Mk, 0), colsum=gkvb, partials=self.S.tn_partials(), defer_fold=_DEFER_FOLD))
+            _tn_group(wgrads)
+            dkvin = _empty((B * HWr, C), dt, dev)
+            dgrads = [ops.gemm_nt_args(dkv, wkvT, dkvin, B * HWr, C, 2 * C, 2 * C, 2 * C, C, a_map=rowmap(HWr, Mk, 0))]
+            if not lin_fuse:
+                dgrads.insert(0, ops.gemm_nt_args(dq, self.wT(p + "attn.q.weight"), dxn1, M, C, C, C, C, C))
+            _nt_group(dgrads)
             ops.gemm_nt(dkv, wkvT, dxn1, B * T, C, 2 * C, 2 * C, 2 * C, C, a_map=rowmap(T, Mk, HWr), c_map=rowmap(T, N, HW), R=dxn1)
-            ops.gemm_tn(dkv, bs["kvin"], gkvw, B * HWr, 2 * C, C, 2 * C, C, C, a_map=rowmap(HWr, Mk, 0), colsum=gkvb, partials=self.S.tn_partials(), defer_fold=_DEFER_FOLD)
-            dkvin = _empty((B * HWr, C), dt, dev)
-            ops.gemm_nt(dkv, wkvT, dkvin, B * HWr, C, 2 * C, 2 * C, 2 * C, C, a_map=rowmap(HWr, Mk, 0))
             dsr = _empty((B * HWr, C), dt, dev)
             ops.layernorm_bwd(dkvin, bs["sr_pre"], dsr, self.f32(p + "attn.norm.weight"), bs["msr"], bs["rsr"], B * HWr, C, C, C, C,
                               dgamma=self.gl(p + "attn.norm.weight"), dbeta=self.gl(p + "attn.norm.bias"), **self.lnk())
@@ -534,7 +549,10 @@
             conv_wgrad(self.S, p + "attn.sr.weight", dsr, bs["xn1"], B * HWr, C, K, C, C, pm, r * r, C, colsum=self.g(p + "attn.sr.bias"))
             ops.gemm_nt(dsr, self.wKT(p + "attn.sr.weight"), dxn1, B * HWr, K, C, C, C, C, c_map=pm, R=dxn1)
         else:
-            ops.gemm_tn(dkv, bs["xn1"], gkvw, M, 2 * C, C, 2 * C, C, C, colsum=gkvb, partials=self.S.tn_partials(), defer_fold=_DEFER_FOLD)
+            wgrads.append(ops.gemm_tn_args(dkv, bs["xn1"], gkvw, M, 2 * C, C, 2 * C, C, C, colsum=gkvb, partials=self.S.tn_partials(), defer_fold=_DEFER_FOLD))
+            _tn_group(wgrads)
+            if not lin_fuse:
+                ops.gemm_nt(dq, self.wT(p + "attn.q.weight"), dxn1, M, C, C, C, C, C)
             ops.gemm_nt(dkv, wkvT, dxn1, M, C, 2 * C, 2 * C, 2 * C, C, R=dxn1)
         prev = self.saved[i]["blocks"][j - 1] if j > 0 else None
         pre = prev is not None and not prev.get("fused_mlp", True) and prev.get("s2") is not None and not _NO_DX2
```

After: 13500, median of 6. About the same (+0.2%).
